# 0xPolygonZero/proof-protocol-decoder

Measured on AMD Instinct MI355X. Metric: txn-proofs/sec (whole node), 256-txn synthetic block, higher is better.
Workload: dtype u64 (Goldilocks field)

## Files before the change

include/bpg.h:

```cpp
#ifndef BPG_H
#define BPG_H
#include <stddef.h>
#include <stdint.h>

#ifdef __cplusplus
extern "C" {
#endif

typedef enum {
  BP_OK = 0,
  BP_ERR_ABORTED = -1,
  BP_ERR_INVALID_INPUT = -2,
  BP_ERR_RANGE = -3,
  BP_ERR_DEVICE = -4,
  BP_ERR_VERIFY = -5,
  BP_ERR_UNSUPPORTED = -6
} bp_status;

const char* bp_last_error(void);
const char* bp_version(void);
int bp_device_count(void);
int bp_use_blocking_sync(int device);
int bp_host_wait_mode(int device);


enum { BP_NTT_FWD_BR2NAT = 0, BP_NTT_INV_NAT2BR = 1, BP_NTT_FWD_NAT = 2, BP_NTT_INV_NAT = 3 };
int bp_ntt_batch(uint64_t* d_cols, uint32_t log_n, uint32_t n_cols, uint64_t col_stride, int dir,
                 void* stream);

int bp_intt_batch(const uint64_t* d_values, uint64_t in_stride, uint64_t* d_coeffs_out, uint64_t out_stride,
                  uint32_t log_n, uint32_t n_cols, void* stream);

int bp_lde_batch(const uint64_t* d_in, uint64_t in_stride, uint64_t* d_coeffs_out, uint64_t coeffs_stride,
                 uint64_t* d_lde_out, uint64_t lde_stride, uint32_t log_n, uint32_t rate_bits,
                 uint32_t n_cols, int from_coeffs, void* stream);

int bp_debug_copy_u64(const uint64_t* d_in, uint64_t* d_out, uint64_t n, void* stream);

int bp_debug_field_ops(const uint64_t* d_a, const uint64_t* d_b, uint64_t* d_out, uint64_t n, void* stream);

void bp_tune_quad_threshold(uint64_t n_perms);
void bp_tune_merkle_fused(int mode);
void bp_tune_merkle_wide(int log2_parents);
void bp_tune_poseidon_mx(int on);
void bp_tune_poseidon_mx_sets(int sets);
void bp_tune_poseidon_grouped(int mode);
void bp_tune_assume_loaded(int mode);
void bp_tune_rec_batch(int n);
void bp_tune_side_lanes(int n);
void bp_tune_witness_threads(int n);
void bp_tune_host_wait(int mode);
void bp_tune_host_poseidon(int mode);
int bp_debug_poseidon_host(uint64_t* states, size_t n);
void bp_tune_k5_spread(int on);
uint32_t bp_debug_poseidon_group_ops(uint32_t K);
int bp_debug_poseidon_group_tables(uint32_t K, uint32_t r0, uint8_t* out_ops, int32_t* out_cform, int32_t* out_cmain,
                                   int32_t* out_max_plane_sum);

void bp_tune_ntt_split(int mode);
void bp_tune_ntt_persist(int on, int resident_workgroups);
void bp_tune_ntt_mx(int mode);
void bp_tune_ntt_mx_wg_per_cu(int n);
int bp_debug_ntt_mx_tables(int kind, int inverse, uint8_t* out_a, int32_t* out_c, uint64_t* out_tw256,
                           uint64_t* out_tw16);
int bp_debug_poseidon_mx_cin(uint32_t* out);

int bp_poseidon_perm_batch(uint64_t* d_states, uint64_t n, void* stream);

uint64_t bp_merkle_digest_words(uint32_t log_leaves, uint32_t cap_height);
int bp_merkle_commit(const uint64_t* d_lde, uint64_t lde_stride, uint32_t n_cols, uint32_t log_n,
                     uint32_t rate_bits, uint32_t cap_height, uint64_t* d_digests, void* stream);

struct bp_stark_cfg;
typedef struct bp_air_family {
  uint32_t first_index, count;
  uint32_t kind;
  uint32_t degree;
} bp_air_family;
typedef struct bp_air_desc {
  uint32_t air_id;
  char name[24];
  uint32_t fixed_n_cols;
  uint32_t n_const_max;
  uint32_t degree;
  uint32_t n_cols, n_aux;
  uint32_t n_air_constraints, n_ctl_constraints;
  uint32_t n_units;
  uint32_t n_families;
  bp_air_family families[24];
} bp_air_desc;
uint32_t bp_air_count(void);
int bp_air_describe(uint32_t air_id, uint32_t n_cols, uint32_t n_const, uint32_t deg_pow, bp_air_desc* out);

int bp_air_register(const uint64_t* program, size_t n_words, uint32_t* air_id_out);
int bp_air_unregister(uint32_t air_id);
int bp_air_program_digest(uint32_t air_id, uint8_t out[32]);

uint64_t bp_quotient_scratch_words(uint32_t air_id, const struct bp_stark_cfg* shape);
int bp_quotient_eval(uint32_t air_id, const struct bp_stark_cfg* shape, const uint64_t* d_trace_lde,
                     const uint64_t* d_aux_lde, const uint64_t* d_const_lde, const uint64_t ctl[4],
                     const uint64_t alphas[2], uint64_t* d_scratch, uint64_t* d_qvals_out, void* stream);

typedef struct bp_air_violation {
  uint32_t row, constraint, family, kind;
  uint64_t value;
} bp_air_violation;
int bp_air_check_trace(uint32_t air_id, const struct bp_stark_cfg* shape, const uint64_t* d_trace, uint64_t stride,
                       const uint64_t* d_consts, const uint64_t pub[4], uint32_t max_rows, uint64_t* n_violated_rows,
                       uint32_t* rows_out, bp_air_violation* viol_out, uint32_t max_viol, uint32_t* n_viol, void* stream);
int bp_air_check_trace_host(uint32_t air_id, const struct bp_stark_cfg* shape, const uint64_t* trace, uint64_t stride,
                            const uint64_t* consts, const uint64_t pub[4], uint32_t max_rows, uint64_t* n_violated_rows,
                            uint32_t* rows_out, bp_air_violation* viol_out, uint32_t max_viol, uint32_t* n_viol);

int bp_keccak_trace(const uint64_t* d_inputs, uint64_t seed, uint32_t log_n, uint64_t* d_trace_out, void* stream);
int bp_logic_trace(const uint64_t* d_inputs, uint64_t seed, uint32_t log_n, uint64_t* d_trace_out, void* stream);
int bp_memory_trace(const uint64_t* d_inputs, uint64_t seed, uint32_t log_n, uint64_t* d_trace_out, void* stream);
int bp_arithmetic_trace(const uint64_t* d_inputs, uint64_t seed, uint32_t log_n, uint64_t* d_trace_out, void* stream);
int bp_byte_packing_trace(const uint64_t* d_inputs, uint64_t seed, uint32_t log_n, uint64_t* d_trace_out, void* stream);
int bp_keccak_sponge_trace(const uint64_t* d_inputs, uint64_t seed, uint32_t log_n, uint64_t* d_trace_out, void* stream);
int bp_arithmetic_mul_trace(const uint64_t* d_inputs, uint64_t seed, uint32_t log_n, uint64_t* d_trace_out, void* stream);

typedef struct bp_plonk_layout {
// ... 194 lines not shown
```

proof_protocol_decoder_amd/_lib.py:

```python
import ctypes as C
import os

_HERE = os.path.dirname(os.path.abspath(__file__))
_PATH = os.environ.get("BPG_LIBBPG") or os.path.join(_HERE, "lib", "libbpg.so")

BP_OK = 0
STATUS_NAMES = {0: "BP_OK", -1: "BP_ERR_ABORTED", -2: "BP_ERR_INVALID_INPUT", -3: "BP_ERR_RANGE",
                -4: "BP_ERR_DEVICE", -5: "BP_ERR_VERIFY", -6: "BP_ERR_UNSUPPORTED"}


class BpgError(RuntimeError):

    def __init__(self, code, message):
        super().__init__("%s: %s" % (STATUS_NAMES.get(code, str(code)), message))
        self.code = code
        self.message = message


class StarkCfg(C.Structure):
    _fields_ = [(n, C.c_uint32) for n in ("log_n", "n_cols", "n_const", "deg_pow", "rate_bits", "cap_height",
                                           "num_queries", "pow_bits", "arity_bits", "final_poly_bits")]


class AirFamily(C.Structure):
    _fields_ = [(n, C.c_uint32) for n in ("first_index", "count", "kind", "degree")]


class AirDesc(C.Structure):
    _fields_ = ([("air_id", C.c_uint32), ("name", C.c_char * 24)]
                + [(n, C.c_uint32) for n in ("fixed_n_cols", "n_const_max", "degree", "n_cols", "n_aux",
                                             "n_air_constraints", "n_ctl_constraints", "n_units", "n_families")]
                + [("families", AirFamily * 24)])


class AirViolation(C.Structure):
    _fields_ = [(n, C.c_uint32) for n in ("row", "constraint", "family", "kind")] + [("value", C.c_uint64)]


def take_buffer(ptr, length):
    try:
        return C.string_at(ptr, length.value)
    finally:
        lib().bp_free_buffer(ptr)


def lib_path():
    return _PATH


_lib = None


def lib():
    global _lib
    if _lib is not None:
        return _lib
    if not os.path.exists(_PATH):
        raise ImportError(
            "libbpg.so not built at %s -- run `python -c 'import __graft_entry__ as g; g.build()'` "
            "(hipcc --offload-arch=gfx950). There is no CPU fallback for the hot path." % _PATH)
    L = C.CDLL(_PATH)
    vp, u32, u64, i = C.c_void_p, C.c_uint32, C.c_uint64, C.c_int
    L.bp_last_error.restype = C.c_char_p
    L.bp_version.restype = C.c_char_p
    L.bp_device_count.restype = i
    L.bp_ntt_batch.argtypes = [vp, u32, u32, u64, i, vp]
    L.bp_lde_batch.argtypes = [vp, u64, vp, u64, vp, u64, u32, u32, u32, i, vp]
    L.bp_poseidon_perm_batch.argtypes = [vp, u64, vp]
    L.bp_debug_field_ops.argtypes = [vp, vp, vp, u64, vp]
    L.bp_quotient_scratch_words.argtypes = [u32, C.POINTER(StarkCfg)]
    L.bp_quotient_scratch_words.restype = u64
    L.bp_quotient_eval.argtypes = [u32, C.POINTER(StarkCfg), vp, vp, vp, C.POINTER(u64), C.POINTER(u64), vp, vp, vp]
    L.bp_air_count.restype = u32
    L.bp_air_describe.argtypes = [u32, u32, u32, u32, C.POINTER(AirDesc)]
    check_args = [u32, C.POINTER(StarkCfg), vp, u64, vp, C.POINTER(u64), u32, C.POINTER(u64), C.POINTER(u32),
                  C.POINTER(AirViolation), u32, C.POINTER(u32)]
    L.bp_air_check_trace.argtypes = check_args + [vp]
    L.bp_air_check_trace_host.argtypes = check_args
    L.bp_keccak_trace.argtypes = [vp, u64, u32, vp, vp]
    L.bp_logic_trace.argtypes = [vp, u64, u32, vp, vp]
    L.bp_memory_trace.argtypes = [vp, u64, u32, vp, vp]
    L.bp_arithmetic_trace.argtypes = [vp, u64, u32, vp, vp]
    L.bp_byte_packing_trace.argtypes = [vp, u64, u32, vp, vp]
    L.bp_keccak_sponge_trace.argtypes = [vp, u64, u32, vp, vp]
    L.bp_arithmetic_mul_trace.argtypes = [vp, u64, u32, vp, vp]
    L.bp_stark_verify_air.argtypes = [u32, C.POINTER(StarkCfg), C.POINTER(u64), C.c_char_p, C.c_size_t]
    L.bp_stark_prove_air.argtypes = [u32, C.POINTER(StarkCfg), u64, u64, i, C.POINTER(C.POINTER(C.c_uint8)),
                                     C.POINTER(C.c_size_t)]
    L.bp_stark_verify_air_pub.argtypes = [u32, C.POINTER(StarkCfg), C.POINTER(u64), C.POINTER(u64), C.c_char_p, C.c_size_t]
    L.bp_stark_prove_trace.argtypes = [u32, C.POINTER(StarkCfg), vp, u64, vp, C.POINTER(u64), i, C.POINTER(C.POINTER(C.c_uint8)),
                                       C.POINTER(C.c_size_t)]
    L.bp_air_register.argtypes = [vp, C.c_size_t, C.POINTER(u32)]
    L.bp_air_unregister.argtypes = [u32]
    L.bp_air_program_digest.argtypes = [u32, C.c_char_p]
    L.bp_fri_fold.argtypes = [vp, u32, u32, u32, u64, C.POINTER(u64), vp, vp]
    L.bp_openings.argtypes = [vp, u64, u32, u32, C.POINTER(u64), C.POINTER(u64), vp, vp, vp]
    L.bp_pow_grind.argtypes = [C.POINTER(u64), u32, u32, C.POINTER(u64), vp]
    L.bp_merkle_digest_words.argtypes = [u32, u32]
    L.bp_merkle_digest_words.restype = u64
    L.bp_merkle_commit.argtypes = [vp, u64, u32, u32, u32, u32, vp, vp]
    L.bp_stark_prove_synthetic.argtypes = [C.POINTER(StarkCfg), u64, u64, i, C.POINTER(C.POINTER(C.c_uint8)),
                                           C.POINTER(C.c_size_t)]
    L.bp_free_buffer.argtypes = [C.POINTER(C.c_uint8)]
    L.bp_free_buffer.restype = None
    L.bp_tune_quad_threshold.argtypes = [u64]
    L.bp_tune_quad_threshold.restype = None
    L.bp_tune_ntt_mx.argtypes = [i]
    L.bp_tune_ntt_mx.restype = None
    L.bp_tune_ntt_mx_wg_per_cu.argtypes = [i]
    L.bp_tune_ntt_mx_wg_per_cu.restype = None
    L.bp_tune_poseidon_mx.argtypes = [i]
    L.bp_tune_poseidon_mx.restype = None
    L.bp_tune_poseidon_mx_sets.argtypes = [i]
    L.bp_tune_poseidon_mx_sets.restype = None
    _lib = L
    return L


def check(rc):
    if rc != BP_OK:
        raise BpgError(rc, lib().bp_last_error().decode("utf-8", "replace"))
```

proof_protocol_decoder_amd/csrc/gl.hpp:

```cpp
#pragma once
#include <cstdint>
#include <hip/hip_runtime.h>

#define GL_HD __host__ __device__ __forceinline__

namespace gl {

constexpr uint64_t P = 0xFFFFFFFF00000001ULL;
constexpr uint64_t EPS = 0xFFFFFFFFULL;
constexpr uint64_t GENERATOR = 7;
constexpr uint64_t TWO_ADIC_ROOT = 1753635133440165772ULL;
constexpr uint64_t W = 7;

#if defined(__HIP__)
namespace cc {
typedef uint64_t mask;
__device__ __forceinline__ uint64_t mad_co(uint32_t a, uint32_t b, uint64_t c, mask& co) {
  uint64_t d;
  asm("v_mad_u64_u32 %0, %1, %2, %3, %4" : "=v"(d), "=s"(co) : "v"(a), "v"(b), "v"(c));
  return d;
}
__device__ __forceinline__ uint64_t mad_eps_co(uint32_t a, uint64_t c, mask& co) {
  uint64_t d;
  asm("v_mad_u64_u32 %0, %1, %2, -1, %3" : "=v"(d), "=s"(co) : "v"(a), "v"(c));
  return d;
}
__device__ __forceinline__ uint32_t add_co(uint32_t a, uint32_t b, mask& co) {
  uint32_t d;
  asm("v_add_co_u32_e64 %0, %1, %2, %3" : "=v"(d), "=s"(co) : "v"(a), "v"(b));
  return d;
}
__device__ __forceinline__ uint32_t addc_co(uint32_t a, uint32_t b, mask ci, mask& co) {
  uint32_t d;
  asm("s_nop 1\n\tv_addc_co_u32_e64 %0, %1, %2, %3, %4" : "=v"(d), "=s"(co) : "v"(a), "v"(b), "s"(ci));
  return d;
}
__device__ __forceinline__ uint32_t addc0_co(uint32_t a, mask ci, mask& co) {
  uint32_t d;
  asm("s_nop 1\n\tv_addc_co_u32_e64 %0, %1, %2, 0, %3" : "=v"(d), "=s"(co) : "v"(a), "s"(ci));
  return d;
}
__device__ __forceinline__ uint32_t sub_co(uint32_t a, uint32_t b, mask& co) {
  uint32_t d;
  asm("v_sub_co_u32_e64 %0, %1, %2, %3" : "=v"(d), "=s"(co) : "v"(a), "v"(b));
  return d;
}
__device__ __forceinline__ uint32_t subb_co(uint32_t a, uint32_t b, mask ci, mask& co) {
  uint32_t d;
  asm("s_nop 1\n\tv_subb_co_u32_e64 %0, %1, %2, %3, %4" : "=v"(d), "=s"(co) : "v"(a), "v"(b), "s"(ci));
  return d;
}
__device__ __forceinline__ uint32_t subb0_co(uint32_t a, mask ci, mask& co) {
  uint32_t d;
  asm("s_nop 1\n\tv_subbrev_co_u32_e64 %0, %1, 0, %2, %3" : "=v"(d), "=s"(co) : "v"(a), "s"(ci));
  return d;
}
__device__ __forceinline__ uint32_t sel_eps(mask m) {
  uint32_t d;
  asm("s_nop 1\n\tv_cndmask_b32_e64 %0, 0, -1, %1" : "=v"(d) : "s"(m));
  return d;
}
__device__ __forceinline__ uint64_t mk64(uint32_t lo, uint32_t hi) { return ((uint64_t)hi << 32) | lo; }
#include "gl_cc.inc"
}
#endif
GL_HD uint64_t canon(uint64_t a) {
  return a >= P ? a - P : a;
}

GL_HD uint64_t add(uint64_t a, uint64_t b) {
  uint64_t s = a + b;
  return s < b ? s + EPS : s;
}
GL_HD uint64_t sub(uint64_t a, uint64_t b) {
  uint64_t d = a - b;
  return a < b ? d - EPS : d;
}
GL_HD uint64_t addc(uint64_t a, uint64_t b) {
  uint64_t s = a + b;
  return (s < a || s >= P) ? s - P : s;
}
GL_HD uint64_t subc(uint64_t a, uint64_t b) {
  return a >= b ? a - b : a + (P - b);
}
GL_HD uint64_t negc(uint64_t a) {
  return a ? P - a : 0;
}

GL_HD uint64_t reduce128(uint64_t lo, uint64_t hi) {
  uint64_t hh = hi >> 32, hl = hi & EPS;
  uint64_t t0 = lo - hh;
  if (lo < hh) t0 -= EPS;
  uint64_t t1 = (hl << 32) - hl;
  uint64_t r = t0 + t1;
  return r < t1 ? r + EPS : r;
}

GL_HD void mul_wide(uint64_t a, uint64_t b, uint64_t& lo, uint64_t& hi) {
#if defined(__HIP_DEVICE_COMPILE__)
  uint32_t a0 = (uint32_t)a, a1 = (uint32_t)(a >> 32), b0 = (uint32_t)b, b1 = (uint32_t)(b >> 32);
  uint64_t p00 = (uint64_t)a0 * b0;
  uint64_t mid = (uint64_t)a0 * b1 + (p00 >> 32);
  uint64_t mid2 = (uint64_t)a1 * b0 + (uint32_t)mid;
  hi = (uint64_t)a1 * b1 + (mid >> 32) + (mid2 >> 32);
  lo = (mid2 << 32) | (uint32_t)p00;
#else
  unsigned __int128 x = (unsigned __int128)a * b;
// ... 41 lines not shown
    P[i] = (uint64_t)a0 * b0[i];
    M[i] = (uint64_t)a0 * b1;
    Q[i] = (uint64_t)a1[i] * b1;
  }
  cc::mad_co(M, C, a1, b0);
#pragma unroll
  for (int i = 0; i < N; i++) {
    t0[i] = (uint32_t)P[i]; t1[i] = (uint32_t)(P[i] >> 32); m0[i] = (uint32_t)M[i]; m1[i] = (uint32_t)(M[i] >> 32);
    q0[i] = (uint32_t)Q[i]; q1[i] = (uint32_t)(Q[i] >> 32);
  }
  cc::add_co(t1, c1, m0);
  cc::addc_co(m1, c2, q0, c1);
  cc::addc0_cv(q1, C);
#pragma unroll
  for (int i = 0; i < N; i++) P[i] = cc::mk64(t0[i], t1[i]);
  cc::mad_eps_co(P, c3, m1);
#pragma unroll
  for (int i = 0; i < N; i++) { t0[i] = (uint32_t)P[i]; t1[i] = (uint32_t)(P[i] >> 32); }
  cc::subb0_co(t0, b3, c3);
#pragma unroll
  for (int i = 0; i < N; i++) c3[i] &= ~b3[i];
  cc::addc0_cv(t1, c3);
  cc::subb_co(t0, bw, q1, c2);
  cc::subb0_co(t1, bw2, bw);
  cc::addc0_co(t0, b3, bw2);
#pragma unroll
  for (int i = 0; i < N; i++) bw2[i] &= ~b3[i];
  cc::subb0_cv(t1, bw2);
#pragma unroll
  for (int i = 0; i < N; i++) r[i] = cc::mk64(t0[i], t1[i]);
}
#endif
#if defined(__HIP__)
template <int N>
__device__ __forceinline__ void add_n(const uint64_t (&a)[N], const uint64_t (&b)[N], uint64_t (&r)[N]) {
  uint32_t al[N], ah[N], bl[N], bh[N], lo[N], hi[N];
  cc::mask c1[N], c2[N], c3[N];
#pragma unroll
  for (int i = 0; i < N; i++) {
    al[i] = (uint32_t)a[i]; ah[i] = (uint32_t)(a[i] >> 32); bl[i] = (uint32_t)b[i]; bh[i] = (uint32_t)(b[i] >> 32);
  }
  cc::add_co_o(lo, c1, al, bl);
  cc::addc_co_o(hi, c2, ah, bh, c1);
  cc::subb0_co(lo, c3, c2);
#pragma unroll
  for (int i = 0; i < N; i++) c2[i] &= ~c3[i];
  cc::addc0_cv(hi, c2);
#pragma unroll
  for (int i = 0; i < N; i++) r[i] = cc::mk64(lo[i], hi[i]);
}
template <int N>
__device__ __forceinline__ void sub_n(const uint64_t (&a)[N], const uint64_t (&b)[N], uint64_t (&r)[N]) {
  uint32_t al[N], ah[N], bl[N], bh[N], lo[N], hi[N];
  cc::mask b1[N], b2[N], b3[N];
#pragma unroll
  for (int i = 0; i < N; i++) {
    al[i] = (uint32_t)a[i]; ah[i] = (uint32_t)(a[i] >> 32); bl[i] = (uint32_t)b[i]; bh[i] = (uint32_t)(b[i] >> 32);
  }
  cc::sub_co_o(lo, b1, al, bl);
  cc::subb_co_o(hi, b2, ah, bh, b1);
  cc::addc0_co(lo, b3, b2);
#pragma unroll
  for (int i = 0; i < N; i++) b2[i] &= ~b3[i];
  cc::subb0_cv(hi, b2);
#pragma unroll
  for (int i = 0; i < N; i++) r[i] = cc::mk64(lo[i], hi[i]);
}
template <int N>
__device__ __forceinline__ void canon_n(uint64_t (&a)[N]) {
  uint32_t lo[N], hi[N], tl[N], th[N];
  cc::mask k[N], c[N];
#pragma unroll
  for (int i = 0; i < N; i++) {
    lo[i] = (uint32_t)a[i]; hi[i] = (uint32_t)(a[i] >> 32);
  }
  cc::add_m1_co_o(tl, k, lo);
  cc::addc0_co_o(th, c, hi, k);
  cc::sel(lo, tl, c);
  cc::sel(hi, th, c);
#pragma unroll
  for (int i = 0; i < N; i++) a[i] = cc::mk64(lo[i], hi[i]);
}
#endif
#if defined(__HIP__)
struct DotAcc {
  uint64_t p, m, q;
  uint32_t cp, cm, cq;
};
__device__ __forceinline__ DotAcc dot_zero() { return DotAcc{0, 0, 0, 0, 0, 0}; }
__device__ __forceinline__ void dot_mad4(DotAcc (&acc)[4], const uint64_t (&a)[4], const uint64_t (&b)[4]) {
  uint32_t a0[4], a1[4], b0[4], b1[4], cnt[4];
  uint64_t col[4];
  cc::mask c[4], cx[4];
#pragma unroll
  for (int i = 0; i < 4; i++) {
    a0[i] = (uint32_t)a[i]; a1[i] = (uint32_t)(a[i] >> 32); b0[i] = (uint32_t)b[i]; b1[i] = (uint32_t)(b[i] >> 32);
  }
#define BPG_DOT_COL(COL, CNT, X, Y)                                  \
  _Pragma("unroll") for (int i = 0; i < 4; i++) { col[i] = acc[i].COL; cnt[i] = acc[i].CNT; } \
  cc::mad_co(col, c, X, Y);                                           \
  cc::addc0_co(cnt, cx, c);                                           \
  _Pragma("unroll") for (int i = 0; i < 4; i++) { acc[i].COL = col[i]; acc[i].CNT = cnt[i]; }
  BPG_DOT_COL(p, cp, a0, b0)
  BPG_DOT_COL(m, cm, a0, b1)
  BPG_DOT_COL(m, cm, a1, b0)
  BPG_DOT_COL(q, cq, a1, b1)
#undef BPG_DOT_COL
}
GL_HD uint64_t mulc(uint64_t a, uint64_t b);
GL_HD uint64_t addc(uint64_t a, uint64_t b);
__device__ __forceinline__ uint64_t dot_reduce(const DotAcc& d) {
  uint64_t r = canon(d.p);
  r = addc(r, mulc(d.m, (uint64_t)1 << 32));
  r = addc(r, mulc(d.q, EPS));
  r = addc(r, mulc(d.cp, EPS));
  r = subc(r, canon((uint64_t)d.cm));
  r = subc(r, mulc(d.cq, (uint64_t)1 << 32));
  return r;
}
#endif
GL_HD uint64_t sqr(uint64_t a) { return mul(a, a); }
GL_HD uint64_t mulc(uint64_t a, uint64_t b) { return canon(mul(a, b)); }

GL_HD uint64_t pow(uint64_t a, uint64_t e) {
  uint64_t r = 1;
  while (e) {
    if (e & 1) r = mulc(r, a);
    a = mulc(a, a);
    e >>= 1;
  }
  return r;
}
GL_HD uint64_t inv(uint64_t a) {
  auto sq_n = [](uint64_t x, int n) {
    for (int i = 0; i < n; i++) x = mul(x, x);
    return x;
  };
  const uint64_t e1 = a;
  const uint64_t e2 = mul(sq_n(e1, 1), e1);
  const uint64_t e3 = mul(sq_n(e2, 1), e1);
  const uint64_t e6 = mul(sq_n(e3, 3), e3);
  const uint64_t e12 = mul(sq_n(e6, 6), e6);
  const uint64_t e24 = mul(sq_n(e12, 12), e12);
  const uint64_t e30 = mul(sq_n(e24, 6), e6);
  const uint64_t e31 = mul(sq_n(e30, 1), e1);
  const uint64_t hi = sq_n(e31, 1);
  const uint64_t lo = mul(hi, a);
  return mulc(sq_n(hi, 32), lo);
}
GL_HD uint64_t root(unsigned k) {
  uint64_t r = TWO_ADIC_ROOT;
  for (unsigned i = k; i < 32; i++) r = mulc(r, r);
  return r;
}

struct Ext {
  uint64_t c0, c1;
};
GL_HD Ext ext(uint64_t a, uint64_t b = 0) { return Ext{a, b}; }
GL_HD bool eq(Ext a, Ext b) { return a.c0 == b.c0 && a.c1 == b.c1; }
GL_HD Ext add(Ext a, Ext b) { return Ext{addc(a.c0, b.c0), addc(a.c1, b.c1)}; }
GL_HD Ext sub(Ext a, Ext b) { return Ext{subc(a.c0, b.c0), subc(a.c1, b.c1)}; }
GL_HD uint64_t mul7(uint64_t x) {
  const uint64_t p = (uint64_t)(uint32_t)x * 7u;
  const uint64_t m = (x >> 32) * 7u + (p >> 32);
  const uint64_t u = (m << 32) | (uint32_t)p;
// ... 43 lines not shown
```

proof_protocol_decoder_amd/csrc/gl_cc.inc:

```
__device__ __forceinline__ void mad_co(uint64_t (&x)[3], mask (&co)[3], const uint32_t (&a)[3], const uint32_t (&b)[3]) {
  asm("v_mad_u64_u32 %0, %3, %6, %9, %0\n\tv_mad_u64_u32 %1, %4, %7, %10, %1\n\tv_mad_u64_u32 %2, %5, %8, %11, %2"
      : "+v"(x[0]), "+v"(x[1]), "+v"(x[2]), "=&s"(co[0]), "=&s"(co[1]), "=&s"(co[2])
      : "v"(a[0]), "v"(a[1]), "v"(a[2]), "v"(b[0]), "v"(b[1]), "v"(b[2]));
}
__device__ __forceinline__ void mad_eps_co(uint64_t (&x)[3], mask (&co)[3], const uint32_t (&a)[3]) {
  asm("v_mad_u64_u32 %0, %3, %6, -1, %0\n\tv_mad_u64_u32 %1, %4, %7, -1, %1\n\tv_mad_u64_u32 %2, %5, %8, -1, %2"
      : "+v"(x[0]), "+v"(x[1]), "+v"(x[2]), "=&s"(co[0]), "=&s"(co[1]), "=&s"(co[2])
      : "v"(a[0]), "v"(a[1]), "v"(a[2]));
}
__device__ __forceinline__ void add_co(uint32_t (&x)[3], mask (&co)[3], const uint32_t (&b)[3]) {
  asm("v_add_co_u32_e64 %0, %3, %0, %6\n\tv_add_co_u32_e64 %1, %4, %1, %7\n\tv_add_co_u32_e64 %2, %5, %2, %8"
      : "+v"(x[0]), "+v"(x[1]), "+v"(x[2]), "=&s"(co[0]), "=&s"(co[1]), "=&s"(co[2])
      : "v"(b[0]), "v"(b[1]), "v"(b[2]));
}
__device__ __forceinline__ void addc_co(uint32_t (&x)[3], mask (&co)[3], const uint32_t (&b)[3], const mask (&ci)[3]) {
  asm("v_addc_co_u32_e64 %0, %3, %0, %6, %9\n\tv_addc_co_u32_e64 %1, %4, %1, %7, %10\n\tv_addc_co_u32_e64 %2, %5, %2, %8, %11"
      : "+v"(x[0]), "+v"(x[1]), "+v"(x[2]), "=&s"(co[0]), "=&s"(co[1]), "=&s"(co[2])
      : "v"(b[0]), "v"(b[1]), "v"(b[2]), "s"(ci[0]), "s"(ci[1]), "s"(ci[2]));
}
__device__ __forceinline__ void addc0_co(uint32_t (&x)[3], mask (&co)[3], const mask (&ci)[3]) {
  asm("v_addc_co_u32_e64 %0, %3, %0, 0, %6\n\tv_addc_co_u32_e64 %1, %4, %1, 0, %7\n\tv_addc_co_u32_e64 %2, %5, %2, 0, %8"
      : "+v"(x[0]), "+v"(x[1]), "+v"(x[2]), "=&s"(co[0]), "=&s"(co[1]), "=&s"(co[2])
      : "s"(ci[0]), "s"(ci[1]), "s"(ci[2]));
}
// ... 2 lines not shown
      : "+v"(x[0]), "+v"(x[1]), "+v"(x[2]), "=&s"(co[0]), "=&s"(co[1]), "=&s"(co[2])
      : "v"(b[0]), "v"(b[1]), "v"(b[2]));
}
__device__ __forceinline__ void subb_co(uint32_t (&x)[3], mask (&co)[3], const uint32_t (&b)[3], const mask (&ci)[3]) {
  asm("v_subb_co_u32_e64 %0, %3, %0, %6, %9\n\tv_subb_co_u32_e64 %1, %4, %1, %7, %10\n\tv_subb_co_u32_e64 %2, %5, %2, %8, %11"
      : "+v"(x[0]), "+v"(x[1]), "+v"(x[2]), "=&s"(co[0]), "=&s"(co[1]), "=&s"(co[2])
      : "v"(b[0]), "v"(b[1]), "v"(b[2]), "s"(ci[0]), "s"(ci[1]), "s"(ci[2]));
}
__device__ __forceinline__ void subb0_co(uint32_t (&x)[3], mask (&co)[3], const mask (&ci)[3]) {
  asm("v_subbrev_co_u32_e64 %0, %3, 0, %0, %6\n\tv_subbrev_co_u32_e64 %1, %4, 0, %1, %7\n\tv_subbrev_co_u32_e64 %2, %5, 0, %2, %8"
      : "+v"(x[0]), "+v"(x[1]), "+v"(x[2]), "=&s"(co[0]), "=&s"(co[1]), "=&s"(co[2])
      : "s"(ci[0]), "s"(ci[1]), "s"(ci[2]));
}
__device__ __forceinline__ void add_m1_co(uint32_t (&x)[3], mask (&co)[3]) {
  asm("v_add_co_u32_e64 %0, %3, %0, -1\n\tv_add_co_u32_e64 %1, %4, %1, -1\n\tv_add_co_u32_e64 %2, %5, %2, -1"
      : "+v"(x[0]), "+v"(x[1]), "+v"(x[2]), "=&s"(co[0]), "=&s"(co[1]), "=&s"(co[2])
      : );
}
__device__ __forceinline__ void sel(uint32_t (&x)[3], const uint32_t (&b)[3], const mask (&ci)[3]) {
  asm("v_cndmask_b32_e64 %0, %0, %3, %6\n\tv_cndmask_b32_e64 %1, %1, %4, %7\n\tv_cndmask_b32_e64 %2, %2, %5, %8"
      : "+v"(x[0]), "+v"(x[1]), "+v"(x[2])
      : "v"(b[0]), "v"(b[1]), "v"(b[2]), "s"(ci[0]), "s"(ci[1]), "s"(ci[2]));
}
__device__ __forceinline__ void sel_eps(uint32_t (&x)[3], const mask (&ci)[3]) {
  asm("v_cndmask_b32_e64 %0, 0, -1, %3\n\tv_cndmask_b32_e64 %1, 0, -1, %4\n\tv_cndmask_b32_e64 %2, 0, -1, %5"
      : "=&v"(x[0]), "=&v"(x[1]), "=&v"(x[2])
      : "s"(ci[0]), "s"(ci[1]), "s"(ci[2]));
}
__device__ __forceinline__ void addc0_cv(uint32_t (&x)[3], const mask (&ci)[3]) {
  asm("v_addc_co_u32_e64 %0, vcc, %0, 0, %3\n\tv_addc_co_u32_e64 %1, vcc, %1, 0, %4\n\tv_addc_co_u32_e64 %2, vcc, %2, 0, %5"
      : "+v"(x[0]), "+v"(x[1]), "+v"(x[2])
      : "s"(ci[0]), "s"(ci[1]), "s"(ci[2]) : "vcc");
}
__device__ __forceinline__ void addc_cv(uint32_t (&x)[3], const uint32_t (&b)[3], const mask (&ci)[3]) {
  asm("v_addc_co_u32_e64 %0, vcc, %0, %3, %6\n\tv_addc_co_u32_e64 %1, vcc, %1, %4, %7\n\tv_addc_co_u32_e64 %2, vcc, %2, %5, %8"
      : "+v"(x[0]), "+v"(x[1]), "+v"(x[2])
      : "v"(b[0]), "v"(b[1]), "v"(b[2]), "s"(ci[0]), "s"(ci[1]), "s"(ci[2]) : "vcc");
}
__device__ __forceinline__ void subb0_cv(uint32_t (&x)[3], const mask (&ci)[3]) {
  asm("v_subbrev_co_u32_e64 %0, vcc, 0, %0, %3\n\tv_subbrev_co_u32_e64 %1, vcc, 0, %1, %4\n\tv_subbrev_co_u32_e64 %2, vcc, 0, %2, %5"
      : "+v"(x[0]), "+v"(x[1]), "+v"(x[2])
      : "s"(ci[0]), "s"(ci[1]), "s"(ci[2]) : "vcc");
}
__device__ __forceinline__ void mad_eps_cv(uint64_t (&x)[3], const uint32_t (&a)[3]) {
  asm("v_mad_u64_u32 %0, vcc, %3, -1, %0\n\tv_mad_u64_u32 %1, vcc, %4, -1, %1\n\tv_mad_u64_u32 %2, vcc, %5, -1, %2"
      : "+v"(x[0]), "+v"(x[1]), "+v"(x[2])
      : "v"(a[0]), "v"(a[1]), "v"(a[2]) : "vcc");
}
__device__ __forceinline__ void sel_one(uint32_t (&x)[3], const mask (&ci)[3]) {
  asm("v_cndmask_b32_e64 %0, %0, 1, %3\n\tv_cndmask_b32_e64 %1, %1, 1, %4\n\tv_cndmask_b32_e64 %2, %2, 1, %5"
      : "+v"(x[0]), "+v"(x[1]), "+v"(x[2])
      : "s"(ci[0]), "s"(ci[1]), "s"(ci[2]));
}
__device__ __forceinline__ void add_co_o(uint32_t (&x)[3], mask (&co)[3], const uint32_t (&a)[3], const uint32_t (&b)[3]) {
  asm("v_add_co_u32_e64 %0, %3, %6, %9\n\tv_add_co_u32_e64 %1, %4, %7, %10\n\tv_add_co_u32_e64 %2, %5, %8, %11"
      : "=&v"(x[0]), "=&v"(x[1]), "=&v"(x[2]), "=&s"(co[0]), "=&s"(co[1]), "=&s"(co[2])
      : "v"(a[0]), "v"(a[1]), "v"(a[2]), "v"(b[0]), "v"(b[1]), "v"(b[2]));
}
__device__ __forceinline__ void addc_co_o(uint32_t (&x)[3], mask (&co)[3], const uint32_t (&a)[3], const uint32_t (&b)[3], const mask (&ci)[3]) {
  asm("v_addc_co_u32_e64 %0, %3, %6, %9, %12\n\tv_addc_co_u32_e64 %1, %4, %7, %10, %13\n\tv_addc_co_u32_e64 %2, %5, %8, %11, %14"
      : "=&v"(x[0]), "=&v"(x[1]), "=&v"(x[2]), "=&s"(co[0]), "=&s"(co[1]), "=&s"(co[2])
      : "v"(a[0]), "v"(a[1]), "v"(a[2]), "v"(b[0]), "v"(b[1]), "v"(b[2]), "s"(ci[0]), "s"(ci[1]), "s"(ci[2]));
}
__device__ __forceinline__ void sub_co_o(uint32_t (&x)[3], mask (&co)[3], const uint32_t (&a)[3], const uint32_t (&b)[3]) {
  asm("v_sub_co_u32_e64 %0, %3, %6, %9\n\tv_sub_co_u32_e64 %1, %4, %7, %10\n\tv_sub_co_u32_e64 %2, %5, %8, %11"
      : "=&v"(x[0]), "=&v"(x[1]), "=&v"(x[2]), "=&s"(co[0]), "=&s"(co[1]), "=&s"(co[2])
      : "v"(a[0]), "v"(a[1]), "v"(a[2]), "v"(b[0]), "v"(b[1]), "v"(b[2]));
}
__device__ __forceinline__ void subb_co_o(uint32_t (&x)[3], mask (&co)[3], const uint32_t (&a)[3], const uint32_t (&b)[3], const mask (&ci)[3]) {
  asm("v_subb_co_u32_e64 %0, %3, %6, %9, %12\n\tv_subb_co_u32_e64 %1, %4, %7, %10, %13\n\tv_subb_co_u32_e64 %2, %5, %8, %11, %14"
      : "=&v"(x[0]), "=&v"(x[1]), "=&v"(x[2]), "=&s"(co[0]), "=&s"(co[1]), "=&s"(co[2])
      : "v"(a[0]), "v"(a[1]), "v"(a[2]), "v"(b[0]), "v"(b[1]), "v"(b[2]), "s"(ci[0]), "s"(ci[1]), "s"(ci[2]));
}
__device__ __forceinline__ void add_m1_co_o(uint32_t (&x)[3], mask (&co)[3], const uint32_t (&a)[3]) {
  asm("v_add_co_u32_e64 %0, %3, %6, -1\n\tv_add_co_u32_e64 %1, %4, %7, -1\n\tv_add_co_u32_e64 %2, %5, %8, -1"
      : "=&v"(x[0]), "=&v"(x[1]), "=&v"(x[2]), "=&s"(co[0]), "=&s"(co[1]), "=&s"(co[2])
      : "v"(a[0]), "v"(a[1]), "v"(a[2]));
}
__device__ __forceinline__ void addc0_co_o(uint32_t (&x)[3], mask (&co)[3], const uint32_t (&a)[3], const mask (&ci)[3]) {
  asm("v_addc_co_u32_e64 %0, %3, %6, 0, %9\n\tv_addc_co_u32_e64 %1, %4, %7, 0, %10\n\tv_addc_co_u32_e64 %2, %5, %8, 0, %11"
      : "=&v"(x[0]), "=&v"(x[1]), "=&v"(x[2]), "=&s"(co[0]), "=&s"(co[1]), "=&s"(co[2])
      : "v"(a[0]), "v"(a[1]), "v"(a[2]), "s"(ci[0]), "s"(ci[1]), "s"(ci[2]));
}
__device__ __forceinline__ void mad_co(uint64_t (&x)[4], mask (&co)[4], const uint32_t (&a)[4], const uint32_t (&b)[4]) {
  asm("v_mad_u64_u32 %0, %4, %8, %12, %0\n\tv_mad_u64_u32 %1, %5, %9, %13, %1\n\tv_mad_u64_u32 %2, %6, %10, %14, %2\n\tv_mad_u64_u32 %3, %7, %11, %15, %3"
      : "+v"(x[0]), "+v"(x[1]), "+v"(x[2]), "+v"(x[3]), "=&s"(co[0]), "=&s"(co[1]), "=&s"(co[2]), "=&s"(co[3])
      : "v"(a[0]), "v"(a[1]), "v"(a[2]), "v"(a[3]), "v"(b[0]), "v"(b[1]), "v"(b[2]), "v"(b[3]));
}
__device__ __forceinline__ void mad_eps_co(uint64_t (&x)[4], mask (&co)[4], const uint32_t (&a)[4]) {
  asm("v_mad_u64_u32 %0, %4, %8, -1, %0\n\tv_mad_u64_u32 %1, %5, %9, -1, %1\n\tv_mad_u64_u32 %2, %6, %10, -1, %2\n\tv_mad_u64_u32 %3, %7, %11, -1, %3"
      : "+v"(x[0]), "+v"(x[1]), "+v"(x[2]), "+v"(x[3]), "=&s"(co[0]), "=&s"(co[1]), "=&s"(co[2]), "=&s"(co[3])
      : "v"(a[0]), "v"(a[1]), "v"(a[2]), "v"(a[3]));
}
__device__ __forceinline__ void add_co(uint32_t (&x)[4], mask (&co)[4], const uint32_t (&b)[4]) {
  asm("v_add_co_u32_e64 %0, %4, %0, %8\n\tv_add_co_u32_e64 %1, %5, %1, %9\n\tv_add_co_u32_e64 %2, %6, %2, %10\n\tv_add_co_u32_e64 %3, %7, %3, %11"
      : "+v"(x[0]), "+v"(x[1]), "+v"(x[2]), "+v"(x[3]), "=&s"(co[0]), "=&s"(co[1]), "=&s"(co[2]), "=&s"(co[3])
      : "v"(b[0]), "v"(b[1]), "v"(b[2]), "v"(b[3]));
}
__device__ __forceinline__ void addc_co(uint32_t (&x)[4], mask (&co)[4], const uint32_t (&b)[4], const mask (&ci)[4]) {
  asm("v_addc_co_u32_e64 %0, %4, %0, %8, %12\n\tv_addc_co_u32_e64 %1, %5, %1, %9, %13\n\tv_addc_co_u32_e64 %2, %6, %2, %10, %14\n\tv_addc_co_u32_e64 %3, %7, %3, %11, %15"
      : "+v"(x[0]), "+v"(x[1]), "+v"(x[2]), "+v"(x[3]), "=&s"(co[0]), "=&s"(co[1]), "=&s"(co[2]), "=&s"(co[3])
      : "v"(b[0]), "v"(b[1]), "v"(b[2]), "v"(b[3]), "s"(ci[0]), "s"(ci[1]), "s"(ci[2]), "s"(ci[3]));
}
__device__ __forceinline__ void addc0_co(uint32_t (&x)[4], mask (&co)[4], const mask (&ci)[4]) {
  asm("v_addc_co_u32_e64 %0, %4, %0, 0, %8\n\tv_addc_co_u32_e64 %1, %5, %1, 0, %9\n\tv_addc_co_u32_e64 %2, %6, %2, 0, %10\n\tv_addc_co_u32_e64 %3, %7, %3, 0, %11"
      : "+v"(x[0]), "+v"(x[1]), "+v"(x[2]), "+v"(x[3]), "=&s"(co[0]), "=&s"(co[1]), "=&s"(co[2]), "=&s"(co[3])
      : "s"(ci[0]), "s"(ci[1]), "s"(ci[2]), "s"(ci[3]));
}
__device__ __forceinline__ void sub_co(uint32_t (&x)[4], mask (&co)[4], const uint32_t (&b)[4]) {
  asm("v_sub_co_u32_e64 %0, %4, %0, %8\n\tv_sub_co_u32_e64 %1, %5, %1, %9\n\tv_sub_co_u32_e64 %2, %6, %2, %10\n\tv_sub_co_u32_e64 %3, %7, %3, %11"
      : "+v"(x[0]), "+v"(x[1]), "+v"(x[2]), "+v"(x[3]), "=&s"(co[0]), "=&s"(co[1]), "=&s"(co[2]), "=&s"(co[3])
      : "v"(b[0]), "v"(b[1]), "v"(b[2]), "v"(b[3]));
}
__device__ __forceinline__ void subb_co(uint32_t (&x)[4], mask (&co)[4], const uint32_t (&b)[4], const mask (&ci)[4]) {
  asm("v_subb_co_u32_e64 %0, %4, %0, %8, %12\n\tv_subb_co_u32_e64 %1, %5, %1, %9, %13\n\tv_subb_co_u32_e64 %2, %6, %2, %10, %14\n\tv_subb_co_u32_e64 %3, %7, %3, %11, %15"
      : "+v"(x[0]), "+v"(x[1]), "+v"(x[2]), "+v"(x[3]), "=&s"(co[0]), "=&s"(co[1]), "=&s"(co[2]), "=&s"(co[3])
      : "v"(b[0]), "v"(b[1]), "v"(b[2]), "v"(b[3]), "s"(ci[0]), "s"(ci[1]), "s"(ci[2]), "s"(ci[3]));
}
__device__ __forceinline__ void subb0_co(uint32_t (&x)[4], mask (&co)[4], const mask (&ci)[4]) {
  asm("v_subbrev_co_u32_e64 %0, %4, 0, %0, %8\n\tv_subbrev_co_u32_e64 %1, %5, 0, %1, %9\n\tv_subbrev_co_u32_e64 %2, %6, 0, %2, %10\n\tv_subbrev_co_u32_e64 %3, %7, 0, %3, %11"
      : "+v"(x[0]), "+v"(x[1]), "+v"(x[2]), "+v"(x[3]), "=&s"(co[0]), "=&s"(co[1]), "=&s"(co[2]), "=&s"(co[3])
      : "s"(ci[0]), "s"(ci[1]), "s"(ci[2]), "s"(ci[3]));
}
__device__ __forceinline__ void add_m1_co(uint32_t (&x)[4], mask (&co)[4]) {
  asm("v_add_co_u32_e64 %0, %4, %0, -1\n\tv_add_co_u32_e64 %1, %5, %1, -1\n\tv_add_co_u32_e64 %2, %6, %2, -1\n\tv_add_co_u32_e64 %3, %7, %3, -1"
      : "+v"(x[0]), "+v"(x[1]), "+v"(x[2]), "+v"(x[3]), "=&s"(co[0]), "=&s"(co[1]), "=&s"(co[2]), "=&s"(co[3])
      : );
}
__device__ __forceinline__ void sel(uint32_t (&x)[4], const uint32_t (&b)[4], const mask (&ci)[4]) {
  asm("v_cndmask_b32_e64 %0, %0, %4, %8\n\tv_cndmask_b32_e64 %1, %1, %5, %9\n\tv_cndmask_b32_e64 %2, %2, %6, %10\n\tv_cndmask_b32_e64 %3, %3, %7, %11"
      : "+v"(x[0]), "+v"(x[1]), "+v"(x[2]), "+v"(x[3])
      : "v"(b[0]), "v"(b[1]), "v"(b[2]), "v"(b[3]), "s"(ci[0]), "s"(ci[1]), "s"(ci[2]), "s"(ci[3]));
}
__device__ __forceinline__ void sel_eps(uint32_t (&x)[4], const mask (&ci)[4]) {
  asm("v_cndmask_b32_e64 %0, 0, -1, %4\n\tv_cndmask_b32_e64 %1, 0, -1, %5\n\tv_cndmask_b32_e64 %2, 0, -1, %6\n\tv_cndmask_b32_e64 %3, 0, -1, %7"
      : "=&v"(x[0]), "=&v"(x[1]), "=&v"(x[2]), "=&v"(x[3])
      : "s"(ci[0]), "s"(ci[1]), "s"(ci[2]), "s"(ci[3]));
}
__device__ __forceinline__ void addc0_cv(uint32_t (&x)[4], const mask (&ci)[4]) {
  asm("v_addc_co_u32_e64 %0, vcc, %0, 0, %4\n\tv_addc_co_u32_e64 %1, vcc, %1, 0, %5\n\tv_addc_co_u32_e64 %2, vcc, %2, 0, %6\n\tv_addc_co_u32_e64 %3, vcc, %3, 0, %7"
      : "+v"(x[0]), "+v"(x[1]), "+v"(x[2]), "+v"(x[3])
      : "s"(ci[0]), "s"(ci[1]), "s"(ci[2]), "s"(ci[3]) : "vcc");
}
__device__ __forceinline__ void addc_cv(uint32_t (&x)[4], const uint32_t (&b)[4], const mask (&ci)[4]) {
  asm("v_addc_co_u32_e64 %0, vcc, %0, %4, %8\n\tv_addc_co_u32_e64 %1, vcc, %1, %5, %9\n\tv_addc_co_u32_e64 %2, vcc, %2, %6, %10\n\tv_addc_co_u32_e64 %3, vcc, %3, %7, %11"
      : "+v"(x[0]), "+v"(x[1]), "+v"(x[2]), "+v"(x[3])
      : "v"(b[0]), "v"(b[1]), "v"(b[2]), "v"(b[3]), "s"(ci[0]), "s"(ci[1]), "s"(ci[2]), "s"(ci[3]) : "vcc");
}
__device__ __forceinline__ void subb0_cv(uint32_t (&x)[4], const mask (&ci)[4]) {
  asm("v_subbrev_co_u32_e64 %0, vcc, 0, %0, %4\n\tv_subbrev_co_u32_e64 %1, vcc, 0, %1, %5\n\tv_subbrev_co_u32_e64 %2, vcc, 0, %2, %6\n\tv_subbrev_co_u32_e64 %3, vcc, 0, %3, %7"
      : "+v"(x[0]), "+v"(x[1]), "+v"(x[2]), "+v"(x[3])
      : "s"(ci[0]), "s"(ci[1]), "s"(ci[2]), "s"(ci[3]) : "vcc");
}
__device__ __forceinline__ void mad_eps_cv(uint64_t (&x)[4], const uint32_t (&a)[4]) {
  asm("v_mad_u64_u32 %0, vcc, %4, -1, %0\n\tv_mad_u64_u32 %1, vcc, %5, -1, %1\n\tv_mad_u64_u32 %2, vcc, %6, -1, %2\n\tv_mad_u64_u32 %3, vcc, %7, -1, %3"
      : "+v"(x[0]), "+v"(x[1]), "+v"(x[2]), "+v"(x[3])
      : "v"(a[0]), "v"(a[1]), "v"(a[2]), "v"(a[3]) : "vcc");
}
__device__ __forceinline__ void sel_one(uint32_t (&x)[4], const mask (&ci)[4]) {
  asm("v_cndmask_b32_e64 %0, %0, 1, %4\n\tv_cndmask_b32_e64 %1, %1, 1, %5\n\tv_cndmask_b32_e64 %2, %2, 1, %6\n\tv_cndmask_b32_e64 %3, %3, 1, %7"
      : "+v"(x[0]), "+v"(x[1]), "+v"(x[2]), "+v"(x[3])
      : "s"(ci[0]), "s"(ci[1]), "s"(ci[2]), "s"(ci[3]));
}
__device__ __forceinline__ void add_co_o(uint32_t (&x)[4], mask (&co)[4], const uint32_t (&a)[4], const uint32_t (&b)[4]) {
  asm("v_add_co_u32_e64 %0, %4, %8, %12\n\tv_add_co_u32_e64 %1, %5, %9, %13\n\tv_add_co_u32_e64 %2, %6, %10, %14\n\tv_add_co_u32_e64 %3, %7, %11, %15"
      : "=&v"(x[0]), "=&v"(x[1]), "=&v"(x[2]), "=&v"(x[3]), "=&s"(co[0]), "=&s"(co[1]), "=&s"(co[2]), "=&s"(co[3])
      : "v"(a[0]), "v"(a[1]), "v"(a[2]), "v"(a[3]), "v"(b[0]), "v"(b[1]), "v"(b[2]), "v"(b[3]));
}
__device__ __forceinline__ void addc_co_o(uint32_t (&x)[4], mask (&co)[4], const uint32_t (&a)[4], const uint32_t (&b)[4], const mask (&ci)[4]) {
  asm("v_addc_co_u32_e64 %0, %4, %8, %12, %16\n\tv_addc_co_u32_e64 %1, %5, %9, %13, %17\n\tv_addc_co_u32_e64 %2, %6, %10, %14, %18\n\tv_addc_co_u32_e64 %3, %7, %11, %15, %19"
      : "=&v"(x[0]), "=&v"(x[1]), "=&v"(x[2]), "=&v"(x[3]), "=&s"(co[0]), "=&s"(co[1]), "=&s"(co[2]), "=&s"(co[3])
      : "v"(a[0]), "v"(a[1]), "v"(a[2]), "v"(a[3]), "v"(b[0]), "v"(b[1]), "v"(b[2]), "v"(b[3]), "s"(ci[0]), "s"(ci[1]), "s"(ci[2]), "s"(ci[3]));
}
__device__ __forceinline__ void sub_co_o(uint32_t (&x)[4], mask (&co)[4], const uint32_t (&a)[4], const uint32_t (&b)[4]) {
  asm("v_sub_co_u32_e64 %0, %4, %8, %12\n\tv_sub_co_u32_e64 %1, %5, %9, %13\n\tv_sub_co_u32_e64 %2, %6, %10, %14\n\tv_sub_co_u32_e64 %3, %7, %11, %15"
      : "=&v"(x[0]), "=&v"(x[1]), "=&v"(x[2]), "=&v"(x[3]), "=&s"(co[0]), "=&s"(co[1]), "=&s"(co[2]), "=&s"(co[3])
      : "v"(a[0]), "v"(a[1]), "v"(a[2]), "v"(a[3]), "v"(b[0]), "v"(b[1]), "v"(b[2]), "v"(b[3]));
}
__device__ __forceinline__ void subb_co_o(uint32_t (&x)[4], mask (&co)[4], const uint32_t (&a)[4], const uint32_t (&b)[4], const mask (&ci)[4]) {
  asm("v_subb_co_u32_e64 %0, %4, %8, %12, %16\n\tv_subb_co_u32_e64 %1, %5, %9, %13, %17\n\tv_subb_co_u32_e64 %2, %6, %10, %14, %18\n\tv_subb_co_u32_e64 %3, %7, %11, %15, %19"
      : "=&v"(x[0]), "=&v"(x[1]), "=&v"(x[2]), "=&v"(x[3]), "=&s"(co[0]), "=&s"(co[1]), "=&s"(co[2]), "=&s"(co[3])
      : "v"(a[0]), "v"(a[1]), "v"(a[2]), "v"(a[3]), "v"(b[0]), "v"(b[1]), "v"(b[2]), "v"(b[3]), "s"(ci[0]), "s"(ci[1]), "s"(ci[2]), "s"(ci[3]));
}
__device__ __forceinline__ void add_m1_co_o(uint32_t (&x)[4], mask (&co)[4], const uint32_t (&a)[4]) {
  asm("v_add_co_u32_e64 %0, %4, %8, -1\n\tv_add_co_u32_e64 %1, %5, %9, -1\n\tv_add_co_u32_e64 %2, %6, %10, -1\n\tv_add_co_u32_e64 %3, %7, %11, -1"
      : "=&v"(x[0]), "=&v"(x[1]), "=&v"(x[2]), "=&v"(x[3]), "=&s"(co[0]), "=&s"(co[1]), "=&s"(co[2]), "=&s"(co[3])
      : "v"(a[0]), "v"(a[1]), "v"(a[2]), "v"(a[3]));
}
__device__ __forceinline__ void addc0_co_o(uint32_t (&x)[4], mask (&co)[4], const uint32_t (&a)[4], const mask (&ci)[4]) {
  asm("v_addc_co_u32_e64 %0, %4, %8, 0, %12\n\tv_addc_co_u32_e64 %1, %5, %9, 0, %13\n\tv_addc_co_u32_e64 %2, %6, %10, 0, %14\n\tv_addc_co_u32_e64 %3, %7, %11, 0, %15"
      : "=&v"(x[0]), "=&v"(x[1]), "=&v"(x[2]), "=&v"(x[3]), "=&s"(co[0]), "=&s"(co[1]), "=&s"(co[2]), "=&s"(co[3])
      : "v"(a[0]), "v"(a[1]), "v"(a[2]), "v"(a[3]), "s"(ci[0]), "s"(ci[1]), "s"(ci[2]), "s"(ci[3]));
}
```

proof_protocol_decoder_amd/csrc/hash_kernels.hip:

```cpp
#include <atomic>
#include <cstring>
#include <memory>
#include <mutex>
#include <vector>
#include "common.hpp"
#include "poseidon.cuh"
#include "poseidon_mx.cuh"
#include "stark_kernels.hpp"

namespace {

__global__ void __launch_bounds__(256) perm_batch_kernel(uint64_t* __restrict__ states, uint64_t n) {
  uint64_t i = blockIdx.x * (uint64_t)blockDim.x + threadIdx.x;
  if (i >= n) return;
  uint64_t s[12];
#pragma unroll
  for (int k = 0; k < 12; k++) s[k] = states[i * 12 + k];
  poseidon::permute(s);
#pragma unroll
  for (int k = 0; k < 12; k++) states[i * 12 + k] = gl::canon(s[k]);
}

__global__ void __launch_bounds__(256) __attribute__((amdgpu_waves_per_eu(4, 8)))
leaf_hash_kernel(const uint64_t* __restrict__ lde, uint64_t stride, uint32_t n_cols, uint32_t log_n,
// ... 327 lines not shown
        if (mirror && l + 1 == levels) mirror[(wg_first + q) * 4 + c.kb] = d;
        sm[l & 1][q * 4 + c.kb] = d;
      }
    }
    __syncthreads();
    dst += level_parents * 4;
    level_parents >>= 1;
    wg_parents >>= 1;
    wg_first >>= 1;
  }
}

__global__ void __launch_bounds__(256)
merkle_subtree_wide_kernel(const uint64_t* __restrict__ child, uint64_t* __restrict__ out, uint64_t n_parents,
                           uint32_t levels, uint64_t* __restrict__ mirror, uint64_t dig_bstride) {
  if (gridDim.x * gridDim.z <= 64) __builtin_amdgcn_s_setprio(3);
  child += blockIdx.z * dig_bstride;
  out += blockIdx.z * dig_bstride;
  if (mirror) mirror += blockIdx.z * ((n_parents >> (levels - 1)) * 4);
  __shared__ __attribute__((aligned(16))) uint32_t cin[poseidon::mx::CIN_WORDS];
  __shared__ uint64_t sm[2][256 * 4];
  poseidon::mx::build_cin(cin);
  __syncthreads();
  const poseidon::mx::Ctx c = poseidon::mx::make_ctx(cin);
  const uint32_t wave = threadIdx.x >> 6, n = threadIdx.x & 15;
  uint64_t level_parents = n_parents;
  uint32_t wg_parents = n_parents < 256 ? (uint32_t)n_parents : 256u;
  uint64_t wg_first = (uint64_t)blockIdx.x * 256;
  uint64_t* dst = out;
  for (uint32_t l = 0; l < levels; l++) {
    const uint64_t* prev = sm[(l - 1) & 1];
    if (wg_parents >= 64) {
      if (wave * 64 < wg_parents) {
        uint64_t e[4][3];
#pragma unroll
        for (int m = 0; m < 4; m++) {
          const uint32_t q = wave * 64 + 16 * m + n;
          if (l == 0) {
            e[m][0] = child[(wg_first + q) * 8 + c.kb];
            e[m][1] = child[(wg_first + q) * 8 + 4 + c.kb];
          } else {
            e[m][0] = prev[(2 * q) * 4 + c.kb];
            e[m][1] = prev[(2 * q + 1) * 4 + c.kb];
          }
          e[m][2] = 0;
        }
        poseidon::mx::permute<4>(e, c);
#pragma unroll
        for (int m = 0; m < 4; m++) {
          const uint32_t q = wave * 64 + 16 * m + n;
          const uint64_t d = gl::canon(e[m][0]);
          dst[(wg_first + q) * 4 + c.kb] = d;
          if (mirror && l + 1 == levels) mirror[(wg_first + q) * 4 + c.kb] = d;
          sm[l & 1][q * 4 + c.kb] = d;
        }
      }
    } else if (wave * 16 < wg_parents) {
      const uint32_t q = wave * 16 + n, qc = q < wg_parents ? q : wg_parents - 1;
      uint64_t e[1][3];
      if (l == 0) {
        e[0][0] = child[(wg_first + qc) * 8 + c.kb];
        e[0][1] = child[(wg_first + qc) * 8 + 4 + c.kb];
      } else {
        e[0][0] = prev[(2 * qc) * 4 + c.kb];
        e[0][1] = prev[(2 * qc + 1) * 4 + c.kb];
      }
      e[0][2] = 0;
      poseidon::mx::permute<1>(e, c);
      if (q < wg_parents) {
        const uint64_t d = gl::canon(e[0][0]);
        dst[(wg_first + q) * 4 + c.kb] = d;
        if (mirror && l + 1 == levels) mirror[(wg_first + q) * 4 + c.kb] = d;
        sm[l & 1][q * 4 + c.kb] = d;
      }
    }
    __syncthreads();
    dst += level_parents * 4;
    level_parents >>= 1;
    wg_parents >>= 1;
    wg_first >>= 1;
  }
}

__global__ void __launch_bounds__(256)
calib_copy_u64_kernel(const uint64_t* __restrict__ in, uint64_t* __restrict__ out, uint64_t n) {
  uint64_t i = blockIdx.x * (uint64_t)blockDim.x + threadIdx.x;
  const uint64_t stride = (uint64_t)gridDim.x * blockDim.x;
  for (; i < n; i += stride) out[i] = in[i];
}

__global__ void __launch_bounds__(256) field_ops_kernel(const uint64_t* __restrict__ a, const uint64_t* __restrict__ b,
                                                        uint64_t* __restrict__ out, uint64_t n) {
  const uint64_t i0 = (blockIdx.x * (uint64_t)blockDim.x + threadIdx.x) * 4;
  if (i0 >= n) return;
  uint64_t x[4], y[4];
#pragma unroll
  for (int k = 0; k < 4; k++) {
    const uint64_t i = i0 + k < n ? i0 + k : n - 1;
    x[k] = a[i];
    y[k] = b[i];
  }
  uint64_t r4[4], r3[3];
  gl::mul_n<4>(x, y, r4);
  __builtin_amdgcn_sched_barrier(0);
  const uint64_t x3[3] = {x[1], x[2], x[3]}, y3[3] = {y[1], y[2], y[3]};
  gl::mul_n<3>(x3, y3, r3);
  __builtin_amdgcn_sched_barrier(0);
  gl::DotAcc d[4] = {gl::dot_zero(), gl::dot_zero(), gl::dot_zero(), gl::dot_zero()};
  gl::dot_mad4(d, x, y);
  __builtin_amdgcn_sched_barrier(0);
  gl::dot_mad4(d, y, x);
  __builtin_amdgcn_sched_barrier(0);
  const uint64_t yy[4] = {y[0], y[0], y[0], y[0]};
  gl::dot_mad4(d, x, yy);
  __builtin_amdgcn_sched_barrier(0);
  uint64_t cy[4] = {y[0], y[1], y[2], y[3]}, sum4[4], dif4[4], cx4[4] = {x[0], x[1], x[2], x[3]};
  gl::canon_n<4>(cy);
  __builtin_amdgcn_sched_barrier(0);
  gl::add_n<4>(x, cy, sum4);
  __builtin_amdgcn_sched_barrier(0);
  gl::sub_n<4>(x, cy, dif4);
  __builtin_amdgcn_sched_barrier(0);
  gl::canon_n<4>(cx4);
  __builtin_amdgcn_sched_barrier(0);
#pragma unroll
  for (int k = 0; k < 4; k++) {
    const uint64_t i = i0 + k;
    if (i >= n) break;
    const uint64_t cb = gl::canon(y[k]);
    out[0 * n + i] = gl::canon(gl::mul(x[k], y[k]));
    out[1 * n + i] = gl::canon(r4[k]);
    out[2 * n + i] = k ? gl::canon(r3[k - 1]) : gl::canon(r4[0]);
    uint64_t lo, hi;
    gl::mul_wide(x[k], y[k], lo, hi);
    out[3 * n + i] = gl::canon(gl::reduce128(lo, hi));
    out[4 * n + i] = gl::canon(gl::add(x[k], cb));
    out[5 * n + i] = gl::canon(gl::sub(x[k], cb));
    out[6 * n + i] = gl::dot_reduce(d[k]);
    out[7 * n + i] = gl::canon(gl::mul7(x[k]));
    out[8 * n + i] = gl::inv(gl::canon(x[k]));
    const gl::Ext e = gl::mul(gl::Ext{gl::canon(x[k]), cb}, gl::Ext{cb, gl::canon(x[k] ^ y[k])});
    out[9 * n + i] = e.c0;
    out[10 * n + i] = e.c1;
    out[11 * n + i] = gl::canon(sum4[k]);
    out[12 * n + i] = gl::canon(dif4[k]);
    out[13 * n + i] = cx4[k];
    out[14 * n + i] = cy[k];
  }
}

}

namespace bpg {


static std::atomic<uint64_t> g_quad_threshold{0};
static bool g_poseidon_mx_on();
static std::atomic<int> g_active_provers{0};
void prover_active(int delta) { g_active_provers.fetch_add(delta, std::memory_order_relaxed); }
int provers_active() { return g_active_provers.load(std::memory_order_relaxed); }
static std::atomic<int> g_assume_loaded{-1};
bool device_loaded() {
  const int a = g_assume_loaded.load(std::memory_order_relaxed);
  return a < 0 ? g_active_provers.load(std::memory_order_relaxed) >= 6 : a != 0;
}
uint64_t quad_threshold() {
// ... 110 lines not shown
  uint64_t* lvl = d_digests;
  uint32_t l = log_leaves;
  if (mirrored) *mirrored = false;
  if (batch == 0 || batch > MAX_BATCH) return fail(BP_ERR_INVALID_INPUT, "merkle: batch of %u trees", batch);
  while (l > cap_height) {
    const uint64_t cnt = (uint64_t)1 << l, parents = cnt / 2;
    uint64_t* nxt = lvl + cnt * 4;
    const int fmode = g_merkle_fused.load(std::memory_order_relaxed);
    const uint64_t flimit = fmode >= 8 ? (uint64_t)1 << fmode : 2048;
    const bool fused = parents <= flimit && (parents < quad_threshold() || fmode >= 8) && (fmode > 0 || (fmode < 0 && !device_loaded()));
    const uint64_t wlimit = (uint64_t)1 << g_merkle_wide_log2.load(std::memory_order_relaxed);
    if (!fused && fmode > 0 && poseidon_mx() && parents >= 256 && parents <= wlimit && parents % 256 == 0) {
      uint32_t levels = l - cap_height;
      if (levels > 9) levels = 9;
      uint64_t* mir = (l - levels == cap_height) ? mirror : nullptr;
      merkle_subtree_wide_kernel<<<dim3((uint32_t)(parents / 256), 1, batch), 256, 0, st>>>(lvl, nxt, parents, levels, mir, dig_bstride);
      BPG_LAUNCH_CHECK();
      if (mir && mirrored) *mirrored = true;
      for (uint32_t k = 0; k < levels; k++) {
        lvl += ((uint64_t)1 << l) * 4;
        l--;
      }
      continue;
    }
    if (!fused) {
      uint64_t* mir = (l - 1 == cap_height) ? mirror : nullptr;
      if (const int ns = mx_sets(parents * batch)) {
        BPG_MX_DISPATCH(ns, merkle_level_mx_kernel, parents, batch, lvl, nxt, parents, mir, dig_bstride)
      } else if (parents * batch >= quad_threshold())
        merkle_level_kernel<<<dim3(ceil_div(parents, 256), 1, batch), 256, 0, st>>>(lvl, nxt, parents, mir, dig_bstride);
      else
        merkle_level_quad_kernel<<<dim3(ceil_div(cnt * 2, 256), 1, batch), 256, 0, st>>>(lvl, nxt, parents, mir, dig_bstride);
      BPG_LAUNCH_CHECK();
      if (mir && mirrored) *mirrored = true;
      lvl = nxt;
      l--;
      continue;
    }
    uint32_t levels = l - cap_height;
    const uint32_t wgs = parents >= 64 ? (uint32_t)(parents / 64) : 1;
    uint32_t max_levels = 1;
    for (uint64_t p = parents >= 64 ? 64 : parents; p > 1; p >>= 1) max_levels++;
    if (levels > max_levels) levels = max_levels;
    uint64_t* mir = (l - levels == cap_height) ? mirror : nullptr;
    if (poseidon_mx()) merkle_subtree_mx_kernel<<<dim3(wgs, 1, batch), 256, 0, st>>>(lvl, nxt, parents, levels, mir, dig_bstride);
    else merkle_subtree_quad_kernel<<<dim3(wgs, 1, batch), 256, 0, st>>>(lvl, nxt, parents, levels, mir, dig_bstride);
    BPG_LAUNCH_CHECK();
    if (mir && mirrored) *mirrored = true;
    for (uint32_t k = 0; k < levels; k++) {
      lvl += ((uint64_t)1 << l) * 4;
      l--;
    }
  }
  return BP_OK;
}

int merkle_commit_rows(const uint64_t* d_leaves, uint32_t leaf_len, uint32_t log_leaves, uint32_t cap_height,
                       uint64_t* d_digests, hipStream_t st) {
  uint64_t n = (uint64_t)1 << log_leaves;
  leaf_hash_rows_kernel<<<ceil_div(n, 256), 256, 0, st>>>(d_leaves, leaf_len, n, d_digests);
  BPG_LAUNCH_CHECK();
  return merkle_upper_levels(d_digests, log_leaves, cap_height, st, nullptr, nullptr);
}

}

extern "C" {

int bp_debug_copy_u64(const uint64_t* d_in, uint64_t* d_out, uint64_t n, void* stream) {
  if (!d_in || !d_out) return bpg::fail(BP_ERR_INVALID_INPUT, "bp_debug_copy_u64: null buffer");
  calib_copy_u64_kernel<<<4096, 256, 0, bpg::as_stream(stream)>>>(d_in, d_out, n);
  BPG_LAUNCH_CHECK();
  return BP_OK;
}

int bp_debug_field_ops(const uint64_t* d_a, const uint64_t* d_b, uint64_t* d_out, uint64_t n, void* stream) {
  if (!n) return BP_OK;
  if (!d_a || !d_b || !d_out) return bpg::fail(BP_ERR_INVALID_INPUT, "bp_debug_field_ops: null buffer");
  field_ops_kernel<<<bpg::ceil_div(bpg::ceil_div(n, 4), 256), 256, 0, bpg::as_stream(stream)>>>(d_a, d_b, d_out, n);
  BPG_LAUNCH_CHECK();
  return BP_OK;
}

void bp_tune_merkle_fused(int mode) { bpg::g_merkle_fused.store(mode < 0 ? -1 : (mode >= 8 && mode <= 20 ? mode : (mode != 0))); }
void bp_tune_quad_threshold(uint64_t n_perms) { bpg::g_quad_threshold.store(n_perms); }
void bp_tune_poseidon_mx(int on) { bpg::g_poseidon_mx.store(on != 0); }
int bp_debug_poseidon_mx_cin(uint32_t* out) {
  if (!out) return bpg::fail(BP_ERR_INVALID_INPUT, "bp_debug_poseidon_mx_cin: null buffer");
  static const poseidon::mx::CinTable t = poseidon::mx::make_cin_table();
  for (int i = 0; i < poseidon::mx::CIN_WORDS; i++) out[i] = t.v[i];
  return BP_OK;
}
void bp_tune_merkle_wide(int log2_parents) { bpg::g_merkle_wide_log2.store(log2_parents < 8 || log2_parents > 24 ? 0 : log2_parents); }
void bp_tune_assume_loaded(int mode) { bpg::g_assume_loaded.store(mode < 0 ? -1 : (mode != 0)); }
void bp_tune_poseidon_grouped(int mode) { bpg::g_poseidon_grouped.store(mode == 0 ? 0 : (mode == 2 ? 2 : 3)); }

uint32_t bp_debug_poseidon_group_ops(uint32_t K) { return K >= 2 && K <= 8 ? (uint32_t)poseidon::group::layout((int)K).n_ops : 0; }
int bp_debug_poseidon_group_tables(uint32_t K, uint32_t r0, uint8_t* out_ops, int32_t* out_cform, int32_t* out_cmain,
                                   int32_t* out_max_plane_sum) try {
  if (!out_ops || !out_cform || !out_cmain) return bpg::fail(BP_ERR_INVALID_INPUT, "bp_debug_poseidon_group_tables: null output");
  poseidon::group::Tables t;
  if (!poseidon::group::build((int)K, (int)r0, &t))
    return bpg::fail(BP_ERR_INVALID_INPUT, "bp_debug_poseidon_group_tables: no such group (K=%u r0=%u)", K, r0);
  std::memcpy(out_ops, t.ops.data(), t.ops.size());
  std::memcpy(out_cform, t.cform.data(), t.cform.size() * 4);
  std::memcpy(out_cmain, t.cmain.data(), t.cmain.size() * 4);
  if (out_max_plane_sum) *out_max_plane_sum = t.max_plane_sum;
  return BP_OK;
}
BPG_ABI_CATCH("bp_debug_poseidon_group_tables")

void bp_tune_poseidon_mx_sets(int sets) { bpg::g_mx_sets.store(sets == 1 || sets == 2 || sets == 4 ? sets : 0); }

uint64_t bp_merkle_digest_words(uint32_t log_leaves, uint32_t cap_height) {
  return (((uint64_t)2 << log_leaves) - ((uint64_t)1 << cap_height)) * 4;
}

int bp_poseidon_perm_batch(uint64_t* d_states, uint64_t n, void* stream) try {
  if (!n) return BP_OK;
  if (!d_states) return bpg::fail(BP_ERR_INVALID_INPUT, "bp_poseidon_perm_batch: null buffer");
  hipStream_t st = bpg::as_stream(stream);
  using bpg::ceil_div;
  if (const int ns = bpg::mx_sets(n)) {
    BPG_MX_DISPATCH(ns, perm_batch_mx_kernel, n, 1, d_states, n)
  } else
    perm_batch_kernel<<<bpg::ceil_div(n, 256), 256, 0, st>>>(d_states, n);
  BPG_LAUNCH_CHECK();
  return BP_OK;
}
BPG_ABI_CATCH("bp_poseidon_perm_batch")

int bp_merkle_commit(const uint64_t* d_lde, uint64_t lde_stride, uint32_t n_cols, uint32_t log_n,
                     uint32_t rate_bits, uint32_t cap_height, uint64_t* d_digests, void* stream) try {
  return bpg::merkle_commit_cols(d_lde, lde_stride, n_cols, log_n, rate_bits, cap_height, d_digests,
                                 bpg::as_stream(stream), nullptr, nullptr, 1, 0, 0);
}
BPG_ABI_CATCH("bp_merkle_commit")

}

namespace bpg {

int merkle_commit_cols(const uint64_t* d_lde, uint64_t lde_stride, uint32_t n_cols, uint32_t log_n, uint32_t rate_bits,
                       uint32_t cap_height, uint64_t* d_digests, hipStream_t st, uint64_t* mirror, bool* mirrored,
                       uint32_t batch, uint64_t lde_bstride, uint64_t dig_bstride) {
  const uint32_t log_leaves = log_n + rate_bits;
  if (!d_lde || !d_digests) return fail(BP_ERR_INVALID_INPUT, "bp_merkle_commit: null buffer");
  if (log_leaves > 30 || cap_height > log_leaves || n_cols == 0 || lde_stride < ((uint64_t)1 << log_leaves))
    return fail(BP_ERR_INVALID_INPUT,
                "bp_merkle_commit: bad shape (log_n=%u rate_bits=%u cap_height=%u n_cols=%u stride=%llu)", log_n,
                rate_bits, cap_height, n_cols, (unsigned long long)lde_stride);
  if (batch == 0 || batch > MAX_BATCH) return fail(BP_ERR_INVALID_INPUT, "merkle: batch of %u trees", batch);
  uint64_t rows = (uint64_t)1 << log_leaves;
  {
    KernelTimer kt(PROF_LEAF_HASH, st, n_cols > 4 ? (double)batch * (double)rows * (double)((n_cols + 7) / 8) : 0.0);
    int ns = mx_sets(rows * batch);
    while (ns > 1 && (uint64_t)16 * ns > rows) ns >>= 1;
    if (ns && rows >= 16) {
      BPG_MX_DISPATCH(ns, leaf_hash_mx_kernel, rows, batch, d_lde, lde_stride, n_cols, log_n, rate_bits, d_digests, lde_bstride, dig_bstride)
    } else if (rows * batch < quad_threshold())
      leaf_hash_quad_kernel<<<dim3(ceil_div(rows * 4, 256), 1, batch), 256, 0, st>>>(d_lde, lde_stride, n_cols, log_n, rate_bits,
                                                                               d_digests, lde_bstride, dig_bstride);
    else
      leaf_hash_kernel<<<dim3(ceil_div(rows, 256), 1, batch), 256, 0, st>>>(d_lde, lde_stride, n_cols, log_n, rate_bits, d_digests,
                                                                      lde_bstride, dig_bstride);
  }
// ... 6 lines not shown
```

proof_protocol_decoder_amd/csrc/ntt.hip:

```cpp
#include <atomic>
#include <map>
#include <mutex>
#include <tuple>
#include <cstring>
#include <memory>
#include "common.hpp"
#include "gl.hpp"
#include "mx_arith.cuh"

namespace {

constexpr uint32_t LOG_BLK_MAX = 14;

template <int N>
__device__ __forceinline__ void mul_group(uint64_t (&x)[16], const int (&idx)[4], const uint64_t (&d)[4], const uint64_t (&w)[4]) {
  if constexpr (N == 4) {
    uint64_t r[4];
    gl::mul_n<4>(d, w, r);
#pragma unroll
    for (int i = 0; i < 4; i++) x[idx[i]] = r[i];
  } else if constexpr (N == 3) {
    const uint64_t d3[3] = {d[0], d[1], d[2]}, w3[3] = {w[0], w[1], w[2]};
    uint64_t r[3];
    gl::mul_n<3>(d3, w3, r);
#pragma unroll
    for (int i = 0; i < 3; i++) x[idx[i]] = r[i];
  } else {
#pragma unroll
    for (int i = 0; i < N; i++) x[idx[i]] = gl::mul(d[i], w[i]);
  }
}

template <int LOGR, bool J0 = false>
__device__ __forceinline__ void dif_butterflies(uint64_t (&x)[1 << LOGR], const uint64_t* __restrict__ tw,
                                                uint32_t j, uint32_t log_sub, uint32_t tw_shift) {
  constexpr int R = 1 << LOGR, NB = R / 2;
#pragma unroll
  for (int s = 0; s < LOGR; s++) {
    const int half = R >> (s + 1);
    if constexpr (NB % 4 == 0 && J0 && LOGR == 4) {
      uint64_t dd[NB];
#pragma unroll
      for (int k0 = 0; k0 < NB; k0 += 4) {
        uint64_t a[4], b[4], d[4], r[4];
#pragma unroll
        for (int i = 0; i < 4; i++) {
          const int k = k0 + i, m = (k / half) * 2 * half + (k % half);
          a[i] = x[m];
          b[i] = x[m + half];
        }
        gl::canon_n<4>(b);
        gl::add_n<4>(a, b, r);
        gl::sub_n<4>(a, b, d);
#pragma unroll
        for (int i = 0; i < 4; i++) {
          const int k = k0 + i, m = (k / half) * 2 * half + (k % half);
          x[m] = r[i];
          dd[k] = d[i];
        }
      }
      int cnt = 0;
      int idx[4] = {0, 0, 0, 0};
      uint64_t dv[4] = {0, 0, 0, 0}, wv[4] = {0, 0, 0, 0};
      uint64_t xx[16];
#pragma unroll
      for (int i = 0; i < 16; i++) xx[i] = x[i];
#pragma unroll
      for (int k = 0; k < NB; k++) {
        const int m = (k / half) * 2 * half + (k % half), e = m & (half - 1);
        if (e == 0) {
          xx[m + half] = dd[k];
        } else {
          idx[cnt] = m + half;
          dv[cnt] = dd[k];
          wv[cnt] = tw[(uint32_t)e << (tw_shift + s)];
          cnt++;
          if (cnt == 4) {
            mul_group<4>(xx, idx, dv, wv);
            cnt = 0;
          }
        }
      }
      if (cnt == 3) mul_group<3>(xx, idx, dv, wv);
      else if (cnt == 2) mul_group<2>(xx, idx, dv, wv);
      else if (cnt == 1) mul_group<1>(xx, idx, dv, wv);
#pragma unroll
      for (int i = 0; i < 16; i++) x[i] = xx[i];
    } else if constexpr (NB % 4 == 0) {
#pragma unroll
      for (int k0 = 0; k0 < NB; k0 += 4) {
        uint64_t a[4], b[4], d[4], w[4], r[4];
#pragma unroll
        for (int i = 0; i < 4; i++) {
          const int k = k0 + i, m = (k / half) * 2 * half + (k % half);
          const uint32_t p = j + ((uint32_t)(m & (half - 1)) << log_sub);
          w[i] = tw[p << (tw_shift + s)];
          a[i] = x[m];
          b[i] = x[m + half];
        }
        gl::canon_n<4>(b);
        gl::add_n<4>(a, b, r);
        gl::sub_n<4>(a, b, d);
#pragma unroll
        for (int i = 0; i < 4; i++) {
          const int k = k0 + i, m = (k / half) * 2 * half + (k % half);
          x[m] = r[i];
        }
        gl::mul_n<4>(d, w, r);
#pragma unroll
        for (int i = 0; i < 4; i++) {
          const int k = k0 + i, m = (k / half) * 2 * half + (k % half);
          x[m + half] = r[i];
        }
        if constexpr (LOGR >= 4) __builtin_amdgcn_sched_barrier(0);
      }
    } else {
#pragma unroll
      for (int m = 0; m < R; m++) {
        if (m & half) continue;
        const uint64_t a = x[m], b = gl::canon(x[m + half]);
        x[m] = gl::add(a, b);
        if (J0 && (m & (half - 1)) == 0) {
          x[m + half] = gl::sub(a, b);
        } else {
          const uint32_t p = j + ((uint32_t)(m & (half - 1)) << log_sub);
          x[m + half] = gl::mul(gl::sub(a, b), tw[p << (tw_shift + s)]);
        }
      }
    }
  }
}
template <int LOGR, bool J0 = false>
__device__ __forceinline__ void dit_butterflies(uint64_t (&x)[1 << LOGR], const uint64_t* __restrict__ tw,
                                                uint32_t j, uint32_t log_sub, uint32_t tw_shift) {
  constexpr int R = 1 << LOGR, NB = R / 2;
#pragma unroll
  for (int s = 0; s < LOGR; s++) {
    const int step = 1 << s;
    if constexpr (NB % 4 == 0 && J0 && LOGR == 4) {
      uint64_t xx[16];
#pragma unroll
      for (int i = 0; i < 16; i++) xx[i] = x[i];
      int cnt = 0;
      int idx[4] = {0, 0, 0, 0};
      uint64_t dv[4] = {0, 0, 0, 0}, wv[4] = {0, 0, 0, 0};
#pragma unroll
      for (int k = 0; k < NB; k++) {
        const int m = (k / step) * 2 * step + (k % step), e = m & (step - 1);
        if (e != 0) {
          idx[cnt] = m + step;
          dv[cnt] = x[m + step];
          wv[cnt] = tw[(uint32_t)e << (tw_shift + (LOGR - 1 - s))];
          cnt++;
          if (cnt == 4) {
            mul_group<4>(xx, idx, dv, wv);
            cnt = 0;
          }
        }
      }
      if (cnt == 3) mul_group<3>(xx, idx, dv, wv);
      else if (cnt == 2) mul_group<2>(xx, idx, dv, wv);
      else if (cnt == 1) mul_group<1>(xx, idx, dv, wv);
#pragma unroll
      for (int k0 = 0; k0 < NB; k0 += 4) {
        uint64_t a[4], r[4], hi[4], lo[4];
#pragma unroll
        for (int i = 0; i < 4; i++) {
          const int k = k0 + i, m = (k / step) * 2 * step + (k % step);
          a[i] = xx[m];
          r[i] = xx[m + step];
        }
        gl::canon_n<4>(r);
        gl::add_n<4>(a, r, hi);
        gl::sub_n<4>(a, r, lo);
#pragma unroll
        for (int i = 0; i < 4; i++) {
          const int k = k0 + i, m = (k / step) * 2 * step + (k % step);
          x[m] = hi[i];
          x[m + step] = lo[i];
        }
      }
    } else if constexpr (NB % 4 == 0) {
#pragma unroll
      for (int k0 = 0; k0 < NB; k0 += 4) {
        uint64_t a[4], v[4], w[4], r[4], hi[4], lo[4];
#pragma unroll
        for (int i = 0; i < 4; i++) {
          const int k = k0 + i, m = (k / step) * 2 * step + (k % step);
          const uint32_t p = j + ((uint32_t)(m & (step - 1)) << log_sub);
          w[i] = tw[p << (tw_shift + (LOGR - 1 - s))];
          v[i] = x[m + step];
          a[i] = x[m];
        }
        gl::mul_n<4>(v, w, r);
        gl::canon_n<4>(r);
        gl::add_n<4>(a, r, hi);
        gl::sub_n<4>(a, r, lo);
#pragma unroll
        for (int i = 0; i < 4; i++) {
          const int k = k0 + i, m = (k / step) * 2 * step + (k % step);
          x[m] = hi[i];
          x[m + step] = lo[i];
        }
        if constexpr (LOGR >= 4) __builtin_amdgcn_sched_barrier(0);
      }
    } else {
#pragma unroll
      for (int m = 0; m < R; m++) {
        if (m & step) continue;
        const uint32_t p = j + ((uint32_t)(m & (step - 1)) << log_sub);
        const uint64_t a = x[m];
        const uint64_t t = (J0 && (m & (step - 1)) == 0) ? gl::canon(x[m + step])
                                                         : gl::mulc(x[m + step], tw[p << (tw_shift + (LOGR - 1 - s))]);
        x[m] = gl::add(a, t);
        x[m + step] = gl::sub(a, t);
      }
    }
  }
}

template <int LOGR, bool DIF>
__device__ __forceinline__ void lds_pass(uint64_t* buf, uint32_t log_blk, uint32_t span_log,
                                         const uint64_t* __restrict__ tw) {
  constexpr int R = 1 << LOGR;
  const uint32_t log_sub = span_log - LOGR, sub_mask = (1u << log_sub) - 1;
  const uint32_t n_q = 1u << (log_blk - LOGR);
  for (uint32_t q = threadIdx.x; q < n_q; q += blockDim.x) {
    const uint32_t j = q & sub_mask, blk = q >> log_sub;
    const uint32_t base = (blk << span_log) + j;
    uint64_t x[R];
#pragma unroll
    for (int m = 0; m < R; m++) x[m] = buf[base + ((uint32_t)m << log_sub)];
    if (DIF) dif_butterflies<LOGR>(x, tw, j, log_sub, log_blk - span_log);
    else dit_butterflies<LOGR>(x, tw, j, log_sub, log_blk - span_log);
#pragma unroll
    for (int m = 0; m < R; m++) buf[base + ((uint32_t)m << log_sub)] = x[m];
  }
}

struct LdsNttArgs {
  const uint64_t* in;
  uint64_t in_stride;
  uint64_t* out;
  uint64_t out_stride;
  uint64_t out_coset_stride;
  const uint64_t* tw;
  const uint64_t* scale;
  uint64_t out_scalar;
  uint32_t log_blk;
  uint32_t log_n_total;
};

template <bool DIF>
__global__ void __launch_bounds__(1024) ntt_lds_kernel(LdsNttArgs a) {
  if (gridDim.x * gridDim.y * gridDim.z <= 64) __builtin_amdgcn_s_setprio(3);
  extern __shared__ uint64_t buf[];
  const uint32_t n = 1u << a.log_blk;
  const uint64_t off = (uint64_t)blockIdx.x << a.log_blk;
  const uint64_t* src = a.in + blockIdx.y * a.in_stride + off;
  uint64_t* dst = a.out + blockIdx.y * a.out_stride + blockIdx.z * a.out_coset_stride + off;
  if (!DIF && a.scale) {
    const uint64_t* sc = a.scale + ((uint64_t)blockIdx.z << a.log_n_total) + off;
    for (uint32_t i = threadIdx.x; i < n; i += blockDim.x) buf[i] = gl::mulc(src[i], sc[i]);
  } else {
    for (uint32_t i = threadIdx.x; i < n; i += blockDim.x) buf[i] = src[i];
  }
  __syncthreads();
  const uint32_t rem = a.log_blk % 3;
  if (DIF) {
    uint32_t span = a.log_blk;
    for (; span >= 3 && span > rem; span -= 3) {
      lds_pass<3, true>(buf, a.log_blk, span, a.tw);
      __syncthreads();
    }
    if (rem == 1) lds_pass<1, true>(buf, a.log_blk, 1, a.tw);
    else if (rem == 2) lds_pass<2, true>(buf, a.log_blk, 2, a.tw);
    if (rem) __syncthreads();
  } else {
    if (rem == 1) lds_pass<1, false>(buf, a.log_blk, 1, a.tw);
    else if (rem == 2) lds_pass<2, false>(buf, a.log_blk, 2, a.tw);
    if (rem) __syncthreads();
    for (uint32_t span = rem + 3; span <= a.log_blk; span += 3) {
      lds_pass<3, false>(buf, a.log_blk, span, a.tw);
      __syncthreads();
    }
  }
  if (DIF && a.out_scalar != 1) {
    for (uint32_t i = threadIdx.x; i < n; i += blockDim.x) dst[i] = gl::mulc(buf[i], a.out_scalar);
  } else {
    for (uint32_t i = threadIdx.x; i < n; i += blockDim.x) dst[i] = gl::canon(buf[i]);
  }
}

template <int L>
__device__ __forceinline__ uint32_t swz(uint32_t i) {
  uint32_t x;
  if (L == 14) x = (((i >> 6) & 7u) << 2) ^ ((i >> 9) & 31u);
  else if (L == 13) x = (((i >> 5) & 15u) << 1) ^ ((i >> 9) & 15u);
  else x = (((i >> 8) & 1u) << 4) ^ ((i >> 7) & 1u) ^ (((i >> 9) & 7u) << 1);
  return i ^ x;
}
__device__ __forceinline__ uint32_t insert4(uint32_t t, uint32_t m, uint32_t b) {
  return ((t >> b) << (b + 4)) | (m << b) | (t & ((1u << b) - 1));
}
template <int R, int SH, bool CONTIG, bool DIF>
__device__ __forceinline__ void sub_butterflies(uint64_t (&x)[16], const uint64_t* __restrict__ tw, uint32_t j,
                                                uint32_t j_step_log, uint32_t log_sub, uint32_t tw_shift) {
  constexpr int G = 16 >> R;
#pragma unroll
  for (int g = 0; g < G; g++) {
    uint64_t y[1 << R];
#pragma unroll
    for (int u = 0; u < (1 << R); u++) y[u] = CONTIG ? x[(g << R) + u] : x[g + (u << SH)];
    const uint32_t jj = CONTIG ? 0u : j + ((uint32_t)g << j_step_log);
    if (DIF) dif_butterflies<R, CONTIG>(y, tw, jj, log_sub, tw_shift);
    else dit_butterflies<R, CONTIG>(y, tw, jj, log_sub, tw_shift);
#pragma unroll
    for (int u = 0; u < (1 << R); u++) {
      if (CONTIG) x[(g << R) + u] = y[u];
      else x[g + (u << SH)] = y[u];
    }
  }
}

struct Ntt16Args {
  const uint64_t* in;
  uint64_t in_stride;
  uint64_t* out;
  uint64_t out_stride, out_coset_stride;
  const uint64_t* tw;
  const uint64_t* scale;
  uint64_t out_scalar;
  uint32_t log_n_total, n_cosets, n_units;
  const uint64_t* tw_top;
};


template <int L, int F>
__global__ void __launch_bounds__((1 << L) / 16) ntt16_dif_kernel(Ntt16Args a) {
  if (gridDim.x * gridDim.y * gridDim.z <= 64) __builtin_amdgcn_s_setprio(3);
  extern __shared__ uint64_t buf[];
  constexpr uint32_t T = (1u << L) / 16;
  constexpr int RT = (L % 4 == 0) ? 4 : (L % 4);
  const uint32_t t = threadIdx.x;
  const uint64_t* src;
  uint64_t* dst;
  uint64_t x[16];
  if (F) {
    const uint32_t id = blockIdx.x, k = id >> 3, h = k & 1, unit = (k >> 1) * 8 + (id & 7);
    if (unit >= a.n_units) return;
    const uint32_t log_bpc = a.log_n_total - (L + 1);
    const uint32_t col = unit >> log_bpc, blk = unit & ((1u << log_bpc) - 1);
    const uint64_t off = (uint64_t)blk << (L + 1);
    src = a.in + col * a.in_stride + off;
    dst = a.out + col * a.out_stride + off + ((uint64_t)h << L);
#pragma unroll
    for (int m0 = 0; m0 < 16; m0 += 4) {
      uint64_t lo[4], hi[4], r[4];
#pragma unroll
      for (int i = 0; i < 4; i++) {
        lo[i] = src[(m0 + i) * T + t];
        hi[i] = src[(m0 + i) * T + t + (1u << L)];
      }
      gl::canon_n<4>(hi);
      if (h == 0) {
        gl::add_n<4>(lo, hi, r);
      } else {
        uint64_t d[4], w[4];
        gl::sub_n<4>(lo, hi, d);
#pragma unroll
        for (int i = 0; i < 4; i++) w[i] = a.tw_top[(m0 + i) * T + t];
        gl::mul_n<4>(d, w, r);
      }
#pragma unroll
      for (int i = 0; i < 4; i++) x[m0 + i] = r[i];
    }
  } else {
    const uint64_t off = (uint64_t)blockIdx.x << L;
    src = a.in + blockIdx.y * a.in_stride + off;
    dst = a.out + blockIdx.y * a.out_stride + off;
#pragma unroll
    for (int m = 0; m < 16; m++) x[m] = src[m * T + t];
  }
  dif_butterflies<4>(x, a.tw, t, L - 4, 0);
#pragma unroll
  for (int m = 0; m < 16; m++) buf[swz<L>(m * T + t)] = x[m];
  __syncthreads();
#pragma unroll
  for (int b = L - 8; b > 0; b -= 4) {
#pragma unroll
    for (int m = 0; m < 16; m++) x[m] = buf[swz<L>(insert4(t, m, b))];
    dif_butterflies<4>(x, a.tw, t & ((1u << b) - 1), b, L - (b + 4));
#pragma unroll
    for (int m = 0; m < 16; m++) buf[swz<L>(insert4(t, m, b))] = x[m];
    __syncthreads();
  }
  const uint32_t base = gl::bitrev(t, L - 4) << 4;
#pragma unroll
  for (int m = 0; m < 16; m++) x[m] = buf[swz<L>(base | m)];
  sub_butterflies<RT, 0, true, true>(x, a.tw, 0, 0, 0, L - RT);
#pragma unroll
  for (int m = 0; m < 16; m++) buf[swz<L>(base | m)] = x[m];
  __syncthreads();
  if (a.out_scalar != 1) {
#pragma unroll
    for (int m0 = 0; m0 < 16; m0 += 4) {
      uint64_t v[4], w[4], r[4];
#pragma unroll
      for (int i = 0; i < 4; i++) {
        v[i] = buf[swz<L>((m0 + i) * T + t)];
        w[i] = a.out_scalar;
      }
      gl::mul_n<4>(v, w, r);
      gl::canon_n<4>(r);
#pragma unroll
      for (int i = 0; i < 4; i++) dst[(m0 + i) * T + t] = r[i];
    }
  } else {
#pragma unroll
    for (int m0 = 0; m0 < 16; m0 += 4) {
      uint64_t v[4];
#pragma unroll
      for (int i = 0; i < 4; i++) v[i] = buf[swz<L>((m0 + i) * T + t)];
      gl::canon_n<4>(v);
#pragma unroll
      for (int i = 0; i < 4; i++) dst[(m0 + i) * T + t] = v[i];
    }
  }
}

template <int L, int F>
__global__ void __launch_bounds__((1 << L) / 16) __attribute__((amdgpu_waves_per_eu(4, 8))) ntt16_dit_kernel(Ntt16Args a) {
  if (gridDim.x <= 64) __builtin_amdgcn_s_setprio(3);
  extern __shared__ uint64_t buf[];
  constexpr uint32_t T = (1u << L) / 16;
  constexpr int RT = (L % 4 == 0) ? 4 : (L % 4);
  const uint32_t id = blockIdx.x, k = id >> 3;
  const uint32_t per = a.n_cosets << F;
  const uint32_t ch = k % per, coset = ch >> F, h = F ? (ch & 1) : 0, unit = (k / per) * 8 + (id & 7);
  if (unit >= a.n_units) return;
  const uint32_t log_bpc = a.log_n_total - (L + F);
  const uint32_t col = unit >> log_bpc, blk = unit & ((1u << log_bpc) - 1);
  const uint32_t t = threadIdx.x;
  const uint64_t off = (uint64_t)blk << (L + F);
  const uint64_t* src = a.in + col * a.in_stride + off;
  const uint64_t* tw = a.tw;
  uint64_t x[16];
  const uint32_t base = gl::bitrev(t, L - 4) << 4;
  if (F) {
    const ulonglong2* src2 = reinterpret_cast<const ulonglong2*>(src);
    const ulonglong2* sc2 = a.scale ? reinterpret_cast<const ulonglong2*>(a.scale + ((uint64_t)coset << a.log_n_total) + off) : nullptr;
    constexpr uint32_t BR4[16] = {0, 8, 4, 12, 2, 10, 6, 14, 1, 9, 5, 13, 3, 11, 7, 15};
#pragma unroll
    for (int m0 = 0; m0 < 16; m0 += 4) {
      uint64_t c0[4], c1[4], r[4];
#pragma unroll
      for (int i = 0; i < 4; i++) {
        const ulonglong2 c = src2[(m0 + i) * T + t];
        c0[i] = c.x;
        c1[i] = c.y;
      }
      if (sc2) {
        uint64_t s0[4], s1[4], p0[4], p1[4];
#pragma unroll
        for (int i = 0; i < 4; i++) {
          const ulonglong2 sc = sc2[(m0 + i) * T + t];
          s0[i] = sc.x;
          s1[i] = sc.y;
        }
        gl::mul_n<4>(c0, s0, p0);
        gl::mul_n<4>(c1, s1, p1);
        gl::canon_n<4>(p1);
#pragma unroll
        for (int i = 0; i < 4; i++) { c0[i] = p0[i]; c1[i] = p1[i]; }
      } else {
        gl::canon_n<4>(c1);
      }
      if (h == 0) {
        gl::add_n<4>(c0, c1, r);
      } else {
        uint64_t d[4], w[4];
        gl::sub_n<4>(c0, c1, d);
#pragma unroll
        for (int i = 0; i < 4; i++) w[i] = a.tw_top[base | BR4[m0 + i]];
        gl::mul_n<4>(d, w, r);
      }
#pragma unroll
      for (int i = 0; i < 4; i++) buf[swz<L>((m0 + i) * T + t)] = r[i];
    }
  } else if (a.scale) {
    const uint64_t* sc = a.scale + ((uint64_t)coset << a.log_n_total) + off;
#pragma unroll
    for (int m0 = 0; m0 < 16; m0 += 4) {
      uint64_t v[4], w[4], r[4];
#pragma unroll
      for (int i = 0; i < 4; i++) {
        v[i] = src[(m0 + i) * T + t];
        w[i] = sc[(m0 + i) * T + t];
      }
      gl::mul_n<4>(v, w, r);
#pragma unroll
      for (int i = 0; i < 4; i++) buf[swz<L>((m0 + i) * T + t)] = r[i];
    }
  } else {
#pragma unroll
    for (int m = 0; m < 16; m++) buf[swz<L>(m * T + t)] = src[m * T + t];
  }
  __syncthreads();
#pragma unroll
  for (int m = 0; m < 16; m++) x[m] = buf[swz<L>(base | m)];
  dit_butterflies<4, true>(x, tw, 0, 0, L - 4);
#pragma unroll
  for (int m = 0; m < 16; m++) buf[swz<L>(base | m)] = x[m];
  __syncthreads();
#pragma unroll
  for (int b = 4; b + 4 <= L - RT; b += 4) {
#pragma unroll
    for (int m = 0; m < 16; m++) x[m] = buf[swz<L>(insert4(t, m, b))];
    dit_butterflies<4>(x, tw, t & ((1u << b) - 1), b, L - (b + 4));
#pragma unroll
    for (int m = 0; m < 16; m++) buf[swz<L>(insert4(t, m, b))] = x[m];
    __syncthreads();
  }
  uint32_t t2 = t;
  asm volatile("" : "+v"(t2));
#pragma unroll
  for (int m = 0; m < 16; m++) x[m] = buf[swz<L>(m * T + t2)];
  sub_butterflies<RT, 4 - RT, false, false>(x, tw, t2, L - 4, L - RT, 0);
  uint64_t* dst = a.out + col * a.out_stride + coset * a.out_coset_stride + off;
#pragma unroll
  for (int m0 = 0; m0 < 16; m0 += 4) {
    uint64_t v[4] = {x[m0], x[m0 + 1], x[m0 + 2], x[m0 + 3]};
    gl::canon_n<4>(v);
#pragma unroll
    for (int i = 0; i < 4; i++) {
      if (F) dst[2 * ((m0 + i) * T + t2) + h] = v[i];
      else dst[(m0 + i) * T + t2] = v[i];
    }
  }
}

template <int L>
__global__ void __launch_bounds__((1 << L) / 16) __attribute__((amdgpu_waves_per_eu(4, 4)))
ntt16_dit_persist_kernel(Ntt16Args a, uint32_t n_items) {
  extern __shared__ uint64_t buf[];
  constexpr uint32_t T = (1u << L) / 16;
  constexpr int RT = (L % 4 == 0) ? 4 : (L % 4);
  const uint32_t t = threadIdx.x;
  const uint32_t log_bpc = a.log_n_total - L;
  const uint64_t* tw = a.tw;
  auto source_of = [&](uint32_t id) -> const uint64_t* {
    const uint32_t k = id >> 3, unit = (k / a.n_cosets) * 8 + (id & 7);
    if (id >= n_items || unit >= a.n_units) return nullptr;
    const uint32_t col = unit >> log_bpc, blk = unit & ((1u << log_bpc) - 1);
    return a.in + col * a.in_stride + ((uint64_t)blk << L);
  };
  uint64_t xn[16];
  {
    const uint64_t* s0 = source_of(blockIdx.x);
    if (s0) {
#pragma unroll
      for (int m = 0; m < 16; m++) xn[m] = s0[m * T + t];
    }
  }
  for (uint32_t id = blockIdx.x; id < n_items; id += gridDim.x) {
    const uint32_t k = id >> 3, coset = k % a.n_cosets, unit = (k / a.n_cosets) * 8 + (id & 7);
    const uint64_t* next_src = source_of(id + gridDim.x);
    uint32_t ta = t, tb = t, tc = t;
    asm volatile("" : "+v"(ta));
    if (unit >= a.n_units) {
      if (next_src) {
#pragma unroll
        for (int m = 0; m < 16; m++) xn[m] = next_src[m * T + t];
      }
      continue;
    }
    const uint32_t col = unit >> log_bpc, blk = unit & ((1u << log_bpc) - 1);
    const uint64_t off = (uint64_t)blk << L;
    if (a.scale) {
      const uint64_t* sc = a.scale + ((uint64_t)coset << a.log_n_total) + off;
#pragma unroll
      for (int m0 = 0; m0 < 16; m0 += 4) {
        uint64_t v[4], w[4], r[4];
#pragma unroll
        for (int i = 0; i < 4; i++) {
          v[i] = xn[m0 + i];
          w[i] = sc[(m0 + i) * T + ta];
        }
        gl::mul_n<4>(v, w, r);
#pragma unroll
        for (int i = 0; i < 4; i++) buf[swz<L>((m0 + i) * T + ta)] = r[i];
      }
    } else {
#pragma unroll
      for (int m = 0; m < 16; m++) buf[swz<L>(m * T + ta)] = xn[m];
    }
    __syncthreads();
    asm volatile("" : "+v"(tb));
    const uint32_t base = gl::bitrev(tb, L - 4) << 4;
    uint64_t x[16];
#pragma unroll
    for (int m = 0; m < 16; m++) x[m] = buf[swz<L>(base | m)];
    dit_butterflies<4, true>(x, tw, 0, 0, L - 4);
#pragma unroll
    for (int m = 0; m < 16; m++) buf[swz<L>(base | m)] = x[m];
    __syncthreads();
#pragma unroll
    for (int b = 4; b + 4 <= L - RT; b += 4) {
      asm volatile("" : "+v"(tc));
#pragma unroll
      for (int m = 0; m < 16; m++) x[m] = buf[swz<L>(insert4(tc, m, b))];
      dit_butterflies<4>(x, tw, tc & ((1u << b) - 1), b, L - (b + 4));
#pragma unroll
      for (int m = 0; m < 16; m++) buf[swz<L>(insert4(tc, m, b))] = x[m];
      __syncthreads();
    }
    uint32_t t2 = t;
    asm volatile("" : "+v"(t2));
    if (next_src) {
#pragma unroll
      for (int m = 0; m < 16; m++) xn[m] = next_src[m * T + t2];
    }
#pragma unroll
    for (int m = 0; m < 16; m++) x[m] = buf[swz<L>(m * T + t2)];
    sub_butterflies<RT, 4 - RT, false, false>(x, tw, t2, L - 4, L - RT, 0);
    uint64_t* dst = a.out + col * a.out_stride + coset * a.out_coset_stride + off;
#pragma unroll
    for (int m0 = 0; m0 < 16; m0 += 4) {
      uint64_t v[4] = {x[m0], x[m0 + 1], x[m0 + 2], x[m0 + 3]};
      gl::canon_n<4>(v);
#pragma unroll
      for (int i = 0; i < 4; i++) dst[(m0 + i) * T + t2] = v[i];
    }
  }
}

#include "ntt_mx.cuh"

template <int LOGR, bool DIF>
__global__ void __launch_bounds__(256)
ntt_global_pass_kernel(const uint64_t* in, uint64_t in_stride, uint64_t* out, uint64_t out_stride,
                       uint64_t coset_stride, uint32_t log_n, uint32_t span_log,
                       const uint64_t* __restrict__ tw) {
  constexpr int R = 1 << LOGR;
  const uint32_t log_sub = span_log - LOGR;
  const uint32_t q = blockIdx.x * blockDim.x + threadIdx.x;
  if (q >= (1u << (log_n - LOGR))) return;
  const uint32_t j = q & ((1u << log_sub) - 1), blk = q >> log_sub;
  const uint64_t base = ((uint64_t)blk << span_log) + j;
  const uint64_t* src = in + blockIdx.y * in_stride + blockIdx.z * coset_stride + base;
  uint64_t* dst = out + blockIdx.y * out_stride + blockIdx.z * coset_stride + base;
  uint64_t x[R];
#pragma unroll
  for (int m = 0; m < R; m++) x[m] = src[(uint64_t)m << log_sub];
  if (DIF) dif_butterflies<LOGR>(x, tw, j, log_sub, log_n - span_log);
  else dit_butterflies<LOGR>(x, tw, j, log_sub, log_n - span_log);
  if constexpr (R % 4 == 0) {
#pragma unroll
    for (int m0 = 0; m0 < R; m0 += 4) {
      uint64_t v[4] = {x[m0], x[m0 + 1], x[m0 + 2], x[m0 + 3]};
      gl::canon_n<4>(v);
#pragma unroll
      for (int i = 0; i < 4; i++) dst[(uint64_t)(m0 + i) << log_sub] = v[i];
    }
  } else {
#pragma unroll
    for (int m = 0; m < R; m++) dst[(uint64_t)m << log_sub] = gl::canon(x[m]);
  }
}


template <int A, bool DIF>
__global__ void __launch_bounds__(1 << A)
ntt_tile_kernel(const uint64_t* in, uint64_t in_stride, uint64_t* out, uint64_t out_stride, uint64_t coset_stride,
                uint32_t log_n, uint32_t span_log, const uint64_t* __restrict__ tw) {
  constexpr int R = 1 << A, B = A - 4, R1 = 1 << B, G = 16 / R1;
  __shared__ uint64_t tile[R * 16];
  const uint32_t log_s = span_log - A;
  const uint32_t tiles_per_blk = 1u << (log_s - 4);
  const uint32_t blk = blockIdx.x / tiles_per_blk, s0 = (blockIdx.x % tiles_per_blk) << 4;
  const uint32_t s = threadIdx.x & 15, hi = threadIdx.x >> 4;
  const uint64_t base = ((uint64_t)blk << span_log) + s0 + s;
  const uint64_t* src = in + blockIdx.y * in_stride + blockIdx.z * coset_stride + base;
  uint64_t* dst = out + blockIdx.y * out_stride + blockIdx.z * coset_stride + base;
  const uint32_t j16 = (hi << log_s) + s0 + s;
  uint64_t x[16];
  if (DIF) {
#pragma unroll
    for (int m = 0; m < 16; m++) x[m] = src[(uint64_t)(hi + m * (R / 16)) << log_s];
    dif_butterflies<4>(x, tw, j16, span_log - 4, log_n - span_log);
#pragma unroll
    for (int m = 0; m < 16; m++) tile[(hi + m * (R / 16)) * 16 + s] = x[m];
    __syncthreads();
#pragma unroll
    for (int m = 0; m < 16; m++) x[m] = tile[(hi * 16 + m) * 16 + s];
#pragma unroll
    for (int g = 0; g < G; g++) {
      uint64_t y[R1];
#pragma unroll
      for (int u = 0; u < R1; u++) y[u] = x[g * R1 + u];
      dif_butterflies<B>(y, tw, s0 + s, log_s, log_n - span_log + 4);
#pragma unroll
      for (int u = 0; u < R1; u++) x[g * R1 + u] = y[u];
    }
#pragma unroll
    for (int m0 = 0; m0 < 16; m0 += 4) {
      uint64_t v[4] = {x[m0], x[m0 + 1], x[m0 + 2], x[m0 + 3]};
      gl::canon_n<4>(v);
#pragma unroll
      for (int i = 0; i < 4; i++) dst[(uint64_t)(hi * 16 + m0 + i) << log_s] = v[i];
    }
  } else {
#pragma unroll
    for (int m = 0; m < 16; m++) x[m] = src[(uint64_t)(hi * 16 + m) << log_s];
#pragma unroll
    for (int g = 0; g < G; g++) {
      uint64_t y[R1];
#pragma unroll
      for (int u = 0; u < R1; u++) y[u] = x[g * R1 + u];
      dit_butterflies<B>(y, tw, s0 + s, log_s, log_n - span_log + 4);
#pragma unroll
      for (int u = 0; u < R1; u++) x[g * R1 + u] = y[u];
    }
#pragma unroll
    for (int m = 0; m < 16; m++) tile[(hi * 16 + m) * 16 + s] = x[m];
    __syncthreads();
#pragma unroll
    for (int m = 0; m < 16; m++) x[m] = tile[(hi + m * (R / 16)) * 16 + s];
    dit_butterflies<4>(x, tw, j16, span_log - 4, log_n - span_log);
#pragma unroll
    for (int m0 = 0; m0 < 16; m0 += 4) {
      uint64_t v[4] = {x[m0], x[m0 + 1], x[m0 + 2], x[m0 + 3]};
      gl::canon_n<4>(v);
#pragma unroll
      for (int i = 0; i < 4; i++) dst[(uint64_t)(hi + (m0 + i) * (R / 16)) << log_s] = v[i];
    }
  }
}

__global__ void twiddle_table_kernel(uint64_t* out, uint32_t count, uint64_t w) {
  uint32_t e = blockIdx.x * blockDim.x + threadIdx.x;
  if (e < count) out[e] = gl::pow(w, e);
}
__global__ void coset_scale_table_kernel(uint64_t* out, uint32_t log_n, uint32_t rate_bits, uint64_t w_m,
                                         int inverse) {
  uint32_t pos = blockIdx.x * blockDim.x + threadIdx.x;
  if (pos >= (1u << log_n)) return;
  uint32_t t = blockIdx.y;
  uint64_t g = gl::mulc(gl::GENERATOR, gl::pow(w_m, t));
  if (inverse) g = gl::inv(g);
  out[((uint64_t)t << log_n) + pos] = gl::pow(g, gl::bitrev(pos, log_n));
}
__global__ void bitrev_permute_kernel(uint64_t* cols, uint64_t stride, uint32_t log_n) {
  uint32_t i = blockIdx.x * blockDim.x + threadIdx.x;
  if (i >= (1u << log_n)) return;
  uint32_t j = gl::bitrev(i, log_n);
  if (i < j) {
    uint64_t* c = cols + blockIdx.y * stride;
    uint64_t a = c[i], b = c[j];
    c[i] = b;
    c[j] = a;
  }
}

struct TableKey {
  int dev, kind;
  uint32_t log_n, rate_bits;
  bool operator<(const TableKey& o) const {
    return std::tie(dev, kind, log_n, rate_bits) < std::tie(o.dev, o.kind, o.log_n, o.rate_bits);
  }
};
std::mutex g_table_mu;
std::map<TableKey, uint64_t*> g_tables;

}

namespace bpg {

int get_table(int kind, uint32_t log_n, uint32_t rate_bits, const uint64_t** out) {
  int dev = 0;
  BPG_HIP(hipGetDevice(&dev));
  std::lock_guard<std::mutex> lk(g_table_mu);
  TableKey key{dev, kind, log_n, kind >= 2 ? rate_bits : 0};
  auto it = g_tables.find(key);
  if (it != g_tables.end()) {
    *out = it->second;
    return BP_OK;
  }
  uint64_t* d = nullptr;
  if (kind >= 2) {
    uint64_t count = (uint64_t)1 << (log_n + rate_bits);
    BPG_HIP(hipMalloc(&d, count * 8));
    dim3 grid(ceil_div((uint64_t)1 << log_n, 256), 1u << rate_bits);
    coset_scale_table_kernel<<<grid, 256, 0, 0>>>(d, log_n, rate_bits, gl::root(log_n + rate_bits), kind == 3);
  } else {
    uint32_t count = log_n ? (1u << (log_n - 1)) : 1;
    BPG_HIP(hipMalloc(&d, (uint64_t)count * 8));
    uint64_t w = gl::root(log_n);
    if (kind == 1) w = gl::inv(w);
    twiddle_table_kernel<<<ceil_div(count, 256), 256, 0, 0>>>(d, count, w);
  }
  BPG_LAUNCH_CHECK();
  BPG_HIP(hipStreamSynchronize(0));
  g_tables[key] = d;
  *out = d;
  return BP_OK;
}

bool device_loaded();
static std::atomic<int> g_ntt_mx{3};
static bool use_ntt_mx(uint32_t log_blk, bool dit) {
  const int m = g_ntt_mx.load(std::memory_order_relaxed);
  if (m == 3) return log_blk == 13 && !device_loaded();
  if (m == 4) return !dit && log_blk <= 13;
  if (m == 5) return dit && log_blk <= 13;
  return m == 2 || (m == 1 && log_blk <= 13);
}
static std::mutex g_mx_mu;
static std::map<std::tuple<int, int, int>, mxn::Tables*> g_mx_tabs;
static std::atomic<int> g_mx_wg_per_cu{0};
static uint32_t mx_grid(uint32_t items, uint32_t log_blk) {
  static const int cus = [] {
    int dev = 0, n = 256;
    if (hipGetDevice(&dev) == hipSuccess) (void)hipDeviceGetAttribute(&n, hipDeviceAttributeMultiprocessorCount, dev);
    return n > 0 ? n : 256;
  }();
  int per = g_mx_wg_per_cu.load(std::memory_order_relaxed);
  if (per <= 0) per = log_blk == 12 ? 2 : 1;
  const uint32_t resident = ((uint32_t)cus * per + 7) / 8 * 8;
  return items < resident ? items : resident;
}
static int get_mx_tables(int kind, bool inverse, const mxn::Tables** out) {
  int dev = 0;
  BPG_HIP(hipGetDevice(&dev));
  std::lock_guard<std::mutex> lk(g_mx_mu);
  const auto key = std::make_tuple(dev, kind, inverse ? 1 : 0);
  auto it = g_mx_tabs.find(key);
  if (it != g_mx_tabs.end()) {
    *out = it->second;
    return BP_OK;
  }
  auto host = std::make_unique<mxn::Tables>();
  mxn::build_tables(*host, kind, inverse);
  mxn::Tables* d = nullptr;
  BPG_HIP(hipMalloc(&d, sizeof(mxn::Tables)));
  BPG_HIP(hipMemcpy(d, host.get(), sizeof(mxn::Tables), hipMemcpyHostToDevice));
  g_mx_tabs[key] = d;
  *out = d;
  return BP_OK;
}

struct NttPlan {
  uint32_t log_blk;
  uint32_t tile_bits;
  uint32_t n_reg;
  uint32_t reg_bits[4];
};
static NttPlan plan_ntt(uint32_t log_n) {
  NttPlan p{};
  if (log_n <= LOG_BLK_MAX) { p.log_blk = log_n; return p; }
  if (log_n <= 17) { p.log_blk = log_n <= 16 ? 12 : 13; p.n_reg = 1; p.reg_bits[0] = log_n - p.log_blk; return p; }
  if (log_n <= 20) { p.log_blk = 12; p.tile_bits = log_n - 12; return p; }
  if (log_n <= 22) { p.log_blk = log_n - 8; p.tile_bits = 8; return p; }
  p.log_blk = 14; p.tile_bits = 8;
  uint32_t left = log_n - 22;
  p.n_reg = (left + 3) / 4;
  for (uint32_t i = 0; i < p.n_reg; i++) {
    const uint32_t k = (left + (p.n_reg - i) - 1) / (p.n_reg - i);
    p.reg_bits[i] = k;
    left -= k;
  }
  return p;
}
static uint32_t pick_log_blk(uint32_t log_n) { return plan_ntt(log_n).log_blk; }

static std::atomic<int> g_ntt_persist{0};
static std::atomic<int> g_ntt_persist_wgs{256};
static std::atomic<int> g_ntt_split{0};
static bool use_split(uint32_t log_blk, uint64_t workgroups, const void* src, const void* dst, bool dit) {
  const int mode = g_ntt_split.load(std::memory_order_relaxed);
  if (mode == 1 || log_blk < 13 || src == dst) return false;
  if (mode == 2) return true;
  if (dit) return mode == 3 && log_blk == 13 && workgroups < 512;
  return log_blk == 14 || workgroups < 512;
}

static uint32_t lds_threads(uint32_t log_blk) {
  uint32_t t = log_blk >= 3 ? (1u << (log_blk - 3)) : 1;
  return t < 64 ? 64 : (t > 1024 ? 1024 : t);
}

template <bool DIF>
static int launch_global_passes(const uint64_t* in, uint64_t in_stride, uint64_t* out, uint64_t out_stride,
                                uint64_t coset_stride, uint32_t n_cols, uint32_t n_cosets, uint32_t log_n,
                                uint32_t log_blk, const uint64_t* tw, hipStream_t st) {
  const NttPlan p = plan_ntt(log_n);
  uint32_t spans[8], bits[8], tiled[8], cnt = 0;
  uint32_t span = log_n;
  for (uint32_t i = 0; i < p.n_reg; i++) { spans[cnt] = span; bits[cnt] = p.reg_bits[i]; tiled[cnt] = 0; cnt++; span -= p.reg_bits[i]; }
  if (p.tile_bits) { spans[cnt] = span; bits[cnt] = p.tile_bits; tiled[cnt] = 1; cnt++; span -= p.tile_bits; }
  if (span != log_blk || log_blk != p.log_blk) return fail(BP_ERR_DEVICE, "NTT plan mismatch (log_n=%u)", log_n);
  for (uint32_t idx = 0; idx < cnt; idx++) {
    const uint32_t i = DIF ? idx : cnt - 1 - idx;
    const uint64_t* src = (idx == 0) ? in : out;
    const uint64_t src_stride = (idx == 0) ? in_stride : out_stride;
    if (tiled[i]) {
      const dim3 grid(1u << (log_n - bits[i] - 4), n_cols, n_cosets);
      switch (bits[i]) {
        case 6: ntt_tile_kernel<6, DIF><<<grid, 64, 0, st>>>(src, src_stride, out, out_stride, coset_stride, log_n, spans[i], tw); break;
        case 7: ntt_tile_kernel<7, DIF><<<grid, 128, 0, st>>>(src, src_stride, out, out_stride, coset_stride, log_n, spans[i], tw); break;
        default: ntt_tile_kernel<8, DIF><<<grid, 256, 0, st>>>(src, src_stride, out, out_stride, coset_stride, log_n, spans[i], tw); break;
      }
    } else {
      const dim3 grid(ceil_div((uint64_t)1 << (log_n - bits[i]), 256), n_cols, n_cosets);
      switch (bits[i]) {
        case 1: ntt_global_pass_kernel<1, DIF><<<grid, 256, 0, st>>>(src, src_stride, out, out_stride, coset_stride, log_n, spans[i], tw); break;
        case 2: ntt_global_pass_kernel<2, DIF><<<grid, 256, 0, st>>>(src, src_stride, out, out_stride, coset_stride, log_n, spans[i], tw); break;
        case 3: ntt_global_pass_kernel<3, DIF><<<grid, 256, 0, st>>>(src, src_stride, out, out_stride, coset_stride, log_n, spans[i], tw); break;
        case 4: ntt_global_pass_kernel<4, DIF><<<grid, 256, 0, st>>>(src, src_stride, out, out_stride, coset_stride, log_n, spans[i], tw); break;
        default: return fail(BP_ERR_DEVICE, "NTT plan asks for a %u-stage register pass", bits[i]);
      }
    }
    BPG_LAUNCH_CHECK();
  }
  return BP_OK;
}

int intt_nat2br(const uint64_t* in, uint64_t in_stride, uint64_t* out, uint64_t out_stride, uint32_t log_n,
                uint32_t n_cols, bool inverse, hipStream_t st) {
  if (n_cols == 0) return BP_OK;
  const uint32_t log_blk = pick_log_blk(log_n);
  const uint64_t *tw_n = nullptr, *tw_b = nullptr;
  int rc;
  if ((rc = get_table(inverse ? 1 : 0, log_blk, 0, &tw_b))) return rc;
  const uint64_t* src = in;
  uint64_t src_stride = in_stride;
  if (log_n > LOG_BLK_MAX) {
    if ((rc = get_table(inverse ? 1 : 0, log_n, 0, &tw_n))) return rc;
    if ((rc = launch_global_passes<true>(in, in_stride, out, out_stride, 0, n_cols, 1, log_n, log_blk, tw_n, st))) return rc;
    src = out;
    src_stride = out_stride;
  }
  if (log_blk >= 12) {
    Ntt16Args b{};
    b.in = src; b.in_stride = src_stride; b.out = out; b.out_stride = out_stride; b.out_coset_stride = 0;
    b.tw = tw_b; b.scale = nullptr; b.out_scalar = inverse ? gl::inv((uint64_t)1 << log_n) : 1;
    b.log_n_total = log_n; b.n_cosets = 1; b.n_units = 0;
    KernelTimer kt(PROF_INTT_DIF, st, 16.0 * (double)n_cols * (double)((uint64_t)1 << log_n));
    if (use_ntt_mx(log_blk, false)) {
      const mxn::Tables* tab = nullptr;
      if ((rc = get_mx_tables(0, inverse, &tab))) return rc;
      b.n_units = n_cols << (log_n - log_blk);
      const uint32_t g = mx_grid(b.n_units, log_blk);
      if (log_blk == 12) mxn::ntt_mx_dif_kernel<0><<<g, 256, (8u << 12) + 4 * mxn::C_LDS_WORDS, st>>>(b, tab);
      else if (log_blk == 13) mxn::ntt_mx_dif_kernel<1><<<g, 512, (8u << 13) + 4 * mxn::C_LDS_WORDS, st>>>(b, tab);
      else mxn::ntt_mx_dif_kernel<2><<<g, 512, (8u << 14) + 4 * mxn::C_LDS_WORDS, st>>>(b, tab);
    } else if (use_split(log_blk, (uint64_t)n_cols << (log_n - log_blk), src, out, false)) {
      if ((rc = get_table(inverse ? 1 : 0, log_blk - 1, 0, &b.tw))) return rc;
      b.tw_top = tw_b;
      b.n_units = n_cols << (log_n - log_blk);
      const dim3 grid1((b.n_units + 7) / 8 * 8 * 2);
      if (log_blk == 14) ntt16_dif_kernel<13, 1><<<grid1, 512, 8u << 13, st>>>(b);
      else ntt16_dif_kernel<12, 1><<<grid1, 256, 8u << 12, st>>>(b);
    } else {
      const dim3 grid16(1u << (log_n - log_blk), n_cols);
      if (log_blk == 12) ntt16_dif_kernel<12, 0><<<grid16, 256, 8u << 12, st>>>(b);
      else if (log_blk == 13) ntt16_dif_kernel<13, 0><<<grid16, 512, 8u << 13, st>>>(b);
      else ntt16_dif_kernel<14, 0><<<grid16, 1024, 8u << 14, st>>>(b);
    }
    BPG_LAUNCH_CHECK();
    return BP_OK;
  }
  LdsNttArgs a{};
  a.in = src; a.in_stride = src_stride; a.out = out; a.out_stride = out_stride; a.out_coset_stride = 0;
  a.tw = tw_b; a.scale = nullptr;
  a.out_scalar = inverse ? gl::inv((uint64_t)1 << log_n) : 1;
  a.log_blk = log_blk; a.log_n_total = log_n;
  dim3 grid(1u << (log_n - log_blk), n_cols, 1);
  size_t lds = (size_t)8 << log_blk;
  {
    KernelTimer kt(PROF_INTT_DIF, st, 16.0 * (double)n_cols * (double)((uint64_t)1 << log_n));
    ntt_lds_kernel<true><<<grid, lds_threads(log_blk), lds, st>>>(a);
  }
  BPG_LAUNCH_CHECK();
  return BP_OK;
}

int ntt_br2nat(const uint64_t* in, uint64_t in_stride, uint64_t* out, uint64_t out_stride, uint64_t coset_stride,
               uint32_t log_n, uint32_t n_cols, uint32_t n_cosets, const uint64_t* scale, bool inverse,
               hipStream_t st) {
  if (n_cols == 0) return BP_OK;
  const uint32_t log_blk = pick_log_blk(log_n);
  const uint64_t *tw_n = nullptr, *tw_b = nullptr;
  int rc;
  if ((rc = get_table(inverse ? 1 : 0, log_blk, 0, &tw_b))) return rc;
  if (log_blk >= 12) {
    Ntt16Args b{};
    b.in = in; b.in_stride = in_stride; b.out = out; b.out_stride = out_stride; b.out_coset_stride = coset_stride;
    b.tw = tw_b; b.scale = scale; b.out_scalar = 1; b.log_n_total = log_n; b.n_cosets = n_cosets;
    b.n_units = n_cols << (log_n - log_blk);
    {
      KernelTimer kt(PROF_LDE_DIT, st, 8.0 * (double)n_cols * (double)((uint64_t)1 << log_n) * (1.0 + n_cosets), true);
      if (use_ntt_mx(log_blk, true)) {
        const mxn::Tables* tab = nullptr;
        if ((rc = get_mx_tables(1, inverse, &tab))) return rc;
        const uint32_t g = mx_grid((b.n_units + 7) / 8 * 8 * n_cosets, log_blk);
        if (log_blk == 12) BPG_LAUNCH_TIMED(kt, mxn::ntt_mx_dit_kernel<0>, g, 256, (8u << 12) + 4 * mxn::C_LDS_WORDS, st, b, tab);
        else if (log_blk == 13) BPG_LAUNCH_TIMED(kt, mxn::ntt_mx_dit_kernel<1>, g, 512, (8u << 13) + 4 * mxn::C_LDS_WORDS, st, b, tab);
        else BPG_LAUNCH_TIMED(kt, mxn::ntt_mx_dit_kernel<2>, g, 512, (8u << 14) + 4 * mxn::C_LDS_WORDS, st, b, tab);
      } else if (use_split(log_blk, (uint64_t)b.n_units * n_cosets, in, out, true)) {
        if ((rc = get_table(inverse ? 1 : 0, log_blk - 1, 0, &b.tw))) return rc;
        b.tw_top = tw_b;
        const dim3 grid1((b.n_units + 7) / 8 * 8 * n_cosets * 2);
        if (log_blk == 14) BPG_LAUNCH_TIMED(kt, HIP_KERNEL_NAME(ntt16_dit_kernel<13, 1>), grid1, 512, 8u << 13, st, b);
        else BPG_LAUNCH_TIMED(kt, HIP_KERNEL_NAME(ntt16_dit_kernel<12, 1>), grid1, 256, 8u << 12, st, b);
      } else {
        const dim3 grid16((b.n_units + 7) / 8 * 8 * n_cosets);
        if (log_blk == 12) BPG_LAUNCH_TIMED(kt, HIP_KERNEL_NAME(ntt16_dit_kernel<12, 0>), grid16, 256, 8u << 12, st, b);
        else if (log_blk == 13) BPG_LAUNCH_TIMED(kt, HIP_KERNEL_NAME(ntt16_dit_kernel<13, 0>), grid16, 512, 8u << 13, st, b);
        else {
          const uint32_t items = grid16.x, group = 8 * n_cosets;
          const uint32_t resident = std::max<uint32_t>(group, (uint32_t)g_ntt_persist_wgs.load(std::memory_order_relaxed) / group * group);
          if (g_ntt_persist.load(std::memory_order_relaxed) && items > resident && in != out)
            BPG_LAUNCH_TIMED(kt, HIP_KERNEL_NAME(ntt16_dit_persist_kernel<14>), dim3(resident), 1024, 8u << 14, st, b, items);
          else
            BPG_LAUNCH_TIMED(kt, HIP_KERNEL_NAME(ntt16_dit_kernel<14, 0>), grid16, 1024, 8u << 14, st, b);
        }
      }
    }
    BPG_LAUNCH_CHECK();
  } else {
  LdsNttArgs a{};
  a.in = in; a.in_stride = in_stride; a.out = out; a.out_stride = out_stride; a.out_coset_stride = coset_stride;
  a.tw = tw_b; a.scale = scale; a.out_scalar = 1; a.log_blk = log_blk; a.log_n_total = log_n;
  dim3 grid(1u << (log_n - log_blk), n_cols, n_cosets);
  size_t lds = (size_t)8 << log_blk;
  {
    KernelTimer kt(PROF_LDE_DIT, st, 8.0 * (double)n_cols * (double)((uint64_t)1 << log_n) * (1.0 + n_cosets), true);
    BPG_LAUNCH_TIMED(kt, ntt_lds_kernel<false>, grid, lds_threads(log_blk), lds, st, a);
  }
  BPG_LAUNCH_CHECK();
  }
  if (log_n > LOG_BLK_MAX) {
    if ((rc = get_table(inverse ? 1 : 0, log_n, 0, &tw_n))) return rc;
    if ((rc = launch_global_passes<false>(out, out_stride, out, out_stride, coset_stride, n_cols, n_cosets, log_n,
                                          log_blk, tw_n, st)))
      return rc;
  }
  return BP_OK;
}

int bitrev_permute(uint64_t* cols, uint64_t stride, uint32_t log_n, uint32_t n_cols, hipStream_t st) {
  dim3 grid(ceil_div((uint64_t)1 << log_n, 256), n_cols);
  bitrev_permute_kernel<<<grid, 256, 0, st>>>(cols, stride, log_n);
  BPG_LAUNCH_CHECK();
  return BP_OK;
}

static int init_ntt_kernels_once() {
  BPG_HIP(hipFuncSetAttribute(reinterpret_cast<const void*>(&ntt_lds_kernel<true>),
                              hipFuncAttributeMaxDynamicSharedMemorySize, 8 << LOG_BLK_MAX));
  BPG_HIP(hipFuncSetAttribute(reinterpret_cast<const void*>(&ntt_lds_kernel<false>),
                              hipFuncAttributeMaxDynamicSharedMemorySize, 8 << LOG_BLK_MAX));
  BPG_HIP(hipFuncSetAttribute(reinterpret_cast<const void*>(&ntt16_dif_kernel<14, 0>),
                              hipFuncAttributeMaxDynamicSharedMemorySize, 8 << 14));
  BPG_HIP(hipFuncSetAttribute(reinterpret_cast<const void*>(&ntt16_dit_kernel<14, 0>),
                              hipFuncAttributeMaxDynamicSharedMemorySize, 8 << 14));
  BPG_HIP(hipFuncSetAttribute(reinterpret_cast<const void*>(&ntt16_dit_persist_kernel<14>),
                              hipFuncAttributeMaxDynamicSharedMemorySize, 8 << 14));
  BPG_HIP(hipFuncSetAttribute(reinterpret_cast<const void*>(&ntt16_dif_kernel<13, 0>),
                              hipFuncAttributeMaxDynamicSharedMemorySize, 8 << 13));
  BPG_HIP(hipFuncSetAttribute(reinterpret_cast<const void*>(&ntt16_dit_kernel<13, 0>),
                              hipFuncAttributeMaxDynamicSharedMemorySize, 8 << 13));
  BPG_HIP(hipFuncSetAttribute(reinterpret_cast<const void*>(&mxn::ntt_mx_dif_kernel<1>),
                              hipFuncAttributeMaxDynamicSharedMemorySize, (8 << 13) + 4 * mxn::C_LDS_WORDS));
  BPG_HIP(hipFuncSetAttribute(reinterpret_cast<const void*>(&mxn::ntt_mx_dif_kernel<2>),
                              hipFuncAttributeMaxDynamicSharedMemorySize, (8 << 14) + 4 * mxn::C_LDS_WORDS));
  BPG_HIP(hipFuncSetAttribute(reinterpret_cast<const void*>(&mxn::ntt_mx_dit_kernel<1>),
                              hipFuncAttributeMaxDynamicSharedMemorySize, (8 << 13) + 4 * mxn::C_LDS_WORDS));
  BPG_HIP(hipFuncSetAttribute(reinterpret_cast<const void*>(&mxn::ntt_mx_dit_kernel<2>),
// ... 128 lines not shown
```

proof_protocol_decoder_amd/csrc/stark_kernels.hip:

```cpp
#include "common.hpp"
#include "gl.hpp"
#include "poseidon.cuh"
#include "poseidon_mx.cuh"
#include "stark_kernels.hpp"
#include "quotient_dev.cuh"
#include "air_program.hpp"

namespace {

using gl::Ext;
using namespace bpg::k5;

__device__ __forceinline__ uint64_t splitmix64(uint64_t x) {
  uint64_t z = x + 0x9E3779B97F4A7C15ULL;
  z = (z ^ (z >> 30)) * 0xBF58476D1CE4E5B9ULL;
  z = (z ^ (z >> 27)) * 0x94D049BB133111EBULL;
  return z ^ (z >> 31);
}
__device__ __forceinline__ uint64_t rnd(uint64_t seed, uint64_t col, uint64_t row) {
  return gl::canon(splitmix64(seed ^ (col << 32) ^ row));
}
__device__ __forceinline__ uint64_t pow_e(uint64_t t, uint32_t e) {
  return e == 3 ? gl::mulc(gl::mulc(t, t), t) : t;
}
// ... 993 lines not shown
      e[m][0] = a.values[2 * (base[m] + o0) + comp];
      e[m][1] = a.values[2 * (base[m] + o1) + comp];
    }
    poseidon::mx::permute<NS>(e, c);
  }
#pragma unroll
  for (int m = 0; m < NS; m++) {
    const uint64_t id = id0 + 16 * m;
    if (id < n_leaves) {
      const uint32_t t = (uint32_t)(id >> log_q), m0 = (uint32_t)(id & ((1u << log_q) - 1));
      const uint64_t leaf = gl::bitrev((uint32_t)(t + ((uint64_t)m0 << a.rate_bits)), log_q + a.rate_bits);
      a.digests[leaf * 4 + c.kb] = gl::canon(e[m][0]);
    }
  }
}
__global__ void __launch_bounds__(256) fri_fold_kernel(bpg::BatchOf<bpg::FriLayerArgs> batch) {
  if (gridDim.x * gridDim.y * gridDim.z <= 64) __builtin_amdgcn_s_setprio(3);
  const bpg::FriLayerArgs& a = batch.a[blockIdx.z];
  const uint32_t log_q = a.log_nl - a.arity_bits;
  const uint64_t n_out = (uint64_t)1 << (log_q + a.rate_bits);
  const uint64_t id = blockIdx.x * (uint64_t)blockDim.x + threadIdx.x;
  if (id >= n_out) return;
  const uint32_t t = (uint32_t)(id >> log_q), m0 = (uint32_t)(id & ((1u << log_q) - 1));
  const uint64_t base = ((uint64_t)t << a.log_nl) + m0;
  const uint64_t x_inv = gl::mulc(a.g_t_inv[t], root_pow(a.tw_nl_inv, a.log_nl, m0));
  uint64_t c0[16], c1[16];
#pragma unroll
  for (int j = 0; j < 16; j++) {
    const uint64_t p = base + ((uint64_t)j << log_q);
    c0[j] = a.values[2 * p];
    c1[j] = a.values[2 * p + 1];
  }
#pragma unroll
  for (int s = 0; s < 4; s++) {
    const int half = 8 >> s;
#pragma unroll
    for (int k0 = 0; k0 < 8; k0 += 2) {
      uint64_t d[4], w[4], r[4];
      int mm[2];
#pragma unroll
      for (int i = 0; i < 2; i++) {
        const int k = k0 + i, m = (k / half) * 2 * half + (k % half);
        mm[i] = m;
        const uint64_t wv = a.wa_inv_pow[(m & (half - 1)) << s];
        const uint64_t x0 = c0[m], x1 = c1[m], y0 = c0[m + half], y1 = c1[m + half];
        c0[m] = gl::addc(x0, y0);
        c1[m] = gl::addc(x1, y1);
        d[2 * i] = gl::subc(x0, y0);
        d[2 * i + 1] = gl::subc(x1, y1);
        w[2 * i] = wv;
        w[2 * i + 1] = wv;
      }
      if (half == 1) {
#pragma unroll
        for (int i = 0; i < 4; i++) r[i] = d[i];
      } else {
        gl::mul_n<4>(d, w, r);
#pragma unroll
        for (int i = 0; i < 4; i++) r[i] = gl::canon(r[i]);
        __builtin_amdgcn_sched_barrier(0);
      }
#pragma unroll
      for (int i = 0; i < 2; i++) {
        c0[mm[i] + half] = r[2 * i];
        c1[mm[i] + half] = r[2 * i + 1];
      }
    }
  }
  const Ext bx = gl::scale(a.beta, x_inv);
  Ext acc = gl::ext(0);
#pragma unroll
  for (int i = 15; i >= 0; i--) {
    const int slot = ((i & 1) << 3) | ((i & 2) << 1) | ((i & 4) >> 1) | ((i & 8) >> 3);
    acc = gl::add(gl::mul(acc, bx), Ext{c0[slot], c1[slot]});
  }
  acc = gl::scale(acc, a.arity_inv);
  a.out[2 * id] = acc.c0;
  a.out[2 * id + 1] = acc.c1;
}

__global__ void __launch_bounds__(256) pow_grind_kernel(bpg::BatchOf<bpg::PowArgs> batch, unsigned long long* result) {
  const bpg::PowArgs& a = batch.a[blockIdx.z];
  result += blockIdx.z;
  if (__hip_atomic_load(result, __ATOMIC_RELAXED, __HIP_MEMORY_SCOPE_AGENT) < a.base) return;
  const uint64_t cand = a.base + blockIdx.x * (uint64_t)blockDim.x + threadIdx.x;
  uint64_t s[12];
#pragma unroll
  for (int k = 0; k < 12; k++) s[k] = a.state[k];
  s[a.pos] = cand;
  poseidon::permute(s);
  if ((gl::canon(s[7]) >> (64 - a.bits)) == 0) atomicMin(result, (unsigned long long)cand);
}
template <int GR>
__global__ void __launch_bounds__(256) __attribute__((amdgpu_waves_per_eu(3)))
pow_grind_mx_kernel(bpg::BatchOf<bpg::PowArgs> batch, unsigned long long* result, const uint32_t* __restrict__ gtab) {
  const bpg::PowArgs& a = batch.a[blockIdx.z];
  result += blockIdx.z;
  if (__hip_atomic_load(result, __ATOMIC_RELAXED, __HIP_MEMORY_SCOPE_AGENT) < a.base) return;
  constexpr int NG = GR ? GR : 2;
  __shared__ __attribute__((aligned(16))) uint32_t cin[GR ? poseidon::mx::CIN_GROUPED_WORDS<NG> : poseidon::mx::CIN_WORDS];
  __shared__ __attribute__((aligned(16))) uint32_t gt[GR ? poseidon::mx::grp::TABLE_WORDS<NG> : 4];
  if constexpr (GR != 0) {
    poseidon::mx::build_cin_grouped<NG>(cin);
    poseidon::mx::grp::load_tables<NG>(gt, gtab);
  } else {
    poseidon::mx::build_cin(cin);
  }
  __syncthreads();
  const poseidon::mx::Ctx c = poseidon::mx::make_ctx(cin);
  const uint64_t cand0 = a.base + ((uint64_t)blockIdx.x * 4 + (threadIdx.x >> 6)) * 64 + (threadIdx.x & 15);
  uint64_t e[4][3];
#pragma unroll
  for (int s = 0; s < 3; s++) {
    uint64_t w = a.state[4 * s];
#pragma unroll
    for (int q = 1; q < 4; q++) w = c.kb == (uint32_t)q ? a.state[4 * s + q] : w;
    const bool mine = c.kb + 4 * s == a.pos;
#pragma unroll
    for (int m = 0; m < 4; m++) e[m][s] = mine ? cand0 + 16 * m : w;
  }
  if constexpr (GR != 0) poseidon::mx::permute_grouped<NG>(e, c, gt, gtab);
  else poseidon::mx::permute<4>(e, c);
  if (c.kb == 3) {
#pragma unroll
    for (int m = 0; m < 4; m++)
      if ((gl::canon(e[m][1]) >> (64 - a.bits)) == 0) atomicMin(result, (unsigned long long)(cand0 + 16 * m));
  }
}

__global__ void __launch_bounds__(256) query_initial_kernel(bpg::QueryArgs a) {
  if (gridDim.x * gridDim.y * gridDim.z <= 64) __builtin_amdgcn_s_setprio(3);
  const uint32_t b = blockIdx.x / a.n_queries, q = blockIdx.x % a.n_queries, o = blockIdx.y;
  const uint64_t x = a.x_index[blockIdx.x];
  const bpg::QueryOracle& orc = a.proof[b].oracle[o];
  const uint32_t log_rows = a.log_n + a.rate_bits;
  const uint32_t i = gl::bitrev((uint32_t)x, log_rows);
  const uint64_t pos = ((uint64_t)(i & ((1u << a.rate_bits) - 1)) << a.log_n) + (i >> a.rate_bits);
  uint64_t* out = a.proof[b].out;
  if (o == 0 && threadIdx.x == 0) out[(uint64_t)q * a.query_words] = x;
  uint64_t* w = out + (uint64_t)q * a.query_words + orc.out_offset;
  for (uint32_t c = threadIdx.x; c < orc.n_cols; c += blockDim.x) w[c] = orc.lde[(uint64_t)c * orc.stride + pos];
  w += orc.n_cols;
  const uint32_t depth = log_rows - a.cap_height;
  for (uint32_t k = threadIdx.x; k < depth * 4; k += blockDim.x) {
    const uint32_t lvl = k >> 2;
    const uint64_t off = ((uint64_t)2 << log_rows) - ((uint64_t)2 << (log_rows - lvl));
    w[k] = orc.digests[(off + ((x >> lvl) ^ 1)) * 4 + (k & 3)];
  }
  if (q == 0 && o == a.leaf_oracle && a.proof[b].first_leaf && threadIdx.x < 4) a.proof[b].first_leaf[threadIdx.x] = orc.digests[x * 4 + threadIdx.x];
}
__global__ void __launch_bounds__(64) query_layers_kernel(bpg::QueryLayerArgs a) {
  if (gridDim.x * gridDim.y * gridDim.z <= 64) __builtin_amdgcn_s_setprio(3);
  const uint32_t b = blockIdx.x / a.n_queries, q = blockIdx.x % a.n_queries, l = blockIdx.y;
  const bpg::QueryLayer& L = a.proof[b].layer[l];
  const uint32_t arity = 1u << a.arity_bits;
  const uint64_t leaf = a.x_index[blockIdx.x] >> (a.arity_bits * (l + 1));
  const uint32_t log_q = L.log_nl - a.arity_bits, log_leaves = log_q + a.rate_bits;
  const uint32_t c = gl::bitrev((uint32_t)leaf, log_leaves);
  const uint32_t t = c & ((1u << a.rate_bits) - 1), m0 = c >> a.rate_bits;
  const uint64_t base = ((uint64_t)t << L.log_nl) + m0;
  uint64_t* w = a.proof[b].out + (uint64_t)q * a.query_words + L.out_offset;
  for (uint32_t k = threadIdx.x; k < 2 * arity; k += blockDim.x) {
    const uint32_t jj = gl::bitrev(k >> 1, a.arity_bits);
    w[k] = L.values[2 * (base + ((uint64_t)jj << log_q)) + (k & 1)];
  }
  w += 2 * arity;
  const uint32_t depth = log_leaves - a.cap_height;
  for (uint32_t k = threadIdx.x; k < depth * 4; k += blockDim.x) {
    const uint32_t lvl = k >> 2;
    const uint64_t off = ((uint64_t)2 << log_leaves) - ((uint64_t)2 << (log_leaves - lvl));
    w[k] = L.digests[(off + ((leaf >> lvl) ^ 1)) * 4 + (k & 3)];
  }
}

}

namespace bpg {

int launch_synth_constants(uint64_t* d_out, uint32_t log_n, uint32_t n_const, uint64_t seed, hipStream_t st) {
  uint64_t total = (uint64_t)n_const << log_n;
  if (!total) return BP_OK;
// ... 303 lines not shown
```

proof_protocol_decoder_amd/ops.py:

```python
import ctypes as C

import numpy as np
import torch

from ._lib import StarkCfg, check, lib, take_buffer

NTT_FWD_BR2NAT, NTT_INV_NAT2BR, NTT_FWD_NAT, NTT_INV_NAT = 0, 1, 2, 3


def _stream():
    return torch.cuda.current_stream().cuda_stream


def _require_cuda(t):
    if not t.is_cuda:
        raise ValueError("bpg ops need device tensors (there is no CPU fallback)")
    if t.dtype != torch.int64 or not t.is_contiguous():
        raise ValueError("bpg ops need contiguous int64 tensors holding u64 bit patterns")


def ntt_batch_(cols, direction):
    _require_cuda(cols)
    n_cols, n = cols.shape
    check(lib().bp_ntt_batch(cols.data_ptr(), n.bit_length() - 1, n_cols, n, direction, _stream()))
    return cols


def intt_batch(values, out=None):
    import ctypes as C
    _require_cuda(values)
    n_cols, n = values.shape
    out = torch.empty_like(values) if out is None else out
    L = lib()
    L.bp_intt_batch.argtypes = [C.c_void_p, C.c_uint64, C.c_void_p, C.c_uint64, C.c_uint32, C.c_uint32, C.c_void_p]
    check(L.bp_intt_batch(values.data_ptr(), n, out.data_ptr(), n, n.bit_length() - 1, n_cols, _stream()))
    return out


def lde_batch(inp, rate_bits, from_coeffs=False):
    _require_cuda(inp)
    n_cols, n = inp.shape
    coeffs = torch.empty_like(inp)
    lde = torch.empty((n_cols, n << rate_bits), dtype=torch.int64, device=inp.device)
    check(lib().bp_lde_batch(inp.data_ptr(), n, coeffs.data_ptr(), n, lde.data_ptr(), n << rate_bits,
                             n.bit_length() - 1, rate_bits, n_cols, int(from_coeffs), _stream()))
    return coeffs, lde


def poseidon_perm_batch_(states):
    _require_cuda(states)
    check(lib().bp_poseidon_perm_batch(states.data_ptr(), states.numel() // 12, _stream()))
    return states


def field_ops(a, b):
    _require_cuda(a)
    _require_cuda(b)
    n = a.numel()
    out = torch.empty((15, n), dtype=torch.int64, device=a.device)
    check(lib().bp_debug_field_ops(a.data_ptr(), b.data_ptr(), out.data_ptr(), n, _stream()))
    return out


AIR_SYNTHETIC, AIR_KECCAK_F = 0, 1
KECCAK_COLS = 2431
LOGIC_COLS = 524
MEMORY_COLS = 45
ARITHMETIC_COLS = 309
BYTE_PACKING_COLS = 299
KECCAK_SPONGE_COLS = 2414
ARITHMETIC_MUL_COLS = 1217


def air_describe(air_id, n_cols=0, n_const=0, deg_pow=1):
    from ._lib import AirDesc
    d = AirDesc()
    check(lib().bp_air_describe(air_id, n_cols, n_const, deg_pow, C.byref(d)))
    return d


def air_register(words):
    words = np.ascontiguousarray(words, dtype=np.uint64)
    air_id = C.c_uint32()
    check(lib().bp_air_register(words.ctypes.data, words.size, C.byref(air_id)))
    return air_id.value


def air_unregister(air_id):
    check(lib().bp_air_unregister(air_id))


def air_program_digest(air_id):
    out = C.create_string_buffer(32)
    check(lib().bp_air_program_digest(air_id, out))
    return out.raw


def _table_trace(name, n_cols, in_shape, log_n, seed, inputs, device):
    out = torch.empty((n_cols, 1 << log_n), dtype=torch.int64, device=device)
    if inputs is not None:
        _require_cuda(inputs)
        assert inputs.shape == in_shape
    check(getattr(lib(), "bp_%s_trace" % name)(inputs.data_ptr() if inputs is not None else None, seed, log_n, out.data_ptr(),
                                               _stream()))
    return out


def logic_trace(log_n, seed=0, inputs=None, device="cuda"):
    return _table_trace("logic", LOGIC_COLS, (1 << log_n, 9), log_n, seed, inputs, device)


def memory_trace(log_n, seed=0, inputs=None, device="cuda"):
    return _table_trace("memory", MEMORY_COLS, (1 << log_n, 11), log_n, seed, inputs, device)


def arithmetic_trace(log_n, seed=0, inputs=None, device="cuda"):
    return _table_trace("arithmetic", ARITHMETIC_COLS, (1 << log_n, 9), log_n, seed, inputs, device)


def byte_packing_trace(log_n, seed=0, inputs=None, device="cuda"):
    return _table_trace("byte_packing", BYTE_PACKING_COLS, (1 << log_n, 6), log_n, seed, inputs, device)


def keccak_sponge_trace(log_n, seed=0, inputs=None, device="cuda"):
    return _table_trace("keccak_sponge", KECCAK_SPONGE_COLS, (1 << log_n, 44), log_n, seed, inputs, device)


def arithmetic_mul_trace(log_n, seed=0, inputs=None, device="cuda"):
    return _table_trace("arithmetic_mul", ARITHMETIC_MUL_COLS, (1 << log_n, 9), log_n, seed, inputs, device)


def keccak_trace(log_n, seed=0, inputs=None, device="cuda"):
    return _table_trace("keccak", KECCAK_COLS, (((1 << log_n) + 23) // 24, 25), log_n, seed, inputs, device)


def quotient_eval(cfg, trace_lde, aux_lde, const_lde, ctl, alphas, air_id=AIR_SYNTHETIC):
    _require_cuda(trace_lde)
    _require_cuda(aux_lde)
    if const_lde is not None:
        _require_cuda(const_lde)
    rows = trace_lde.shape[1]
    scratch = torch.empty(int(lib().bp_quotient_scratch_words(air_id, C.byref(cfg))), dtype=torch.int64,
                          device=trace_lde.device)
# ... 165 lines not shown
```

Baseline: 33.85.

## Use shift-based power-of-two twiddles in radix-16 NTT passes with per-layer tables

In the Goldilocks field the 16th roots of unity are powers of two (2^12 steps), so the new code replaces the generic 64-bit multiplies inside each radix-16 butterfly with shift-and-reduce sequences. It adds dif16/dit16 kernels that read a precomputed per-layer twiddle table for the inter-group twiddles, and removes the old J0 grouped-multiply path. The 16-point fast path only applies to the forward LDE and the inverse INTT kernels. The PoW grind kernels also get an earlier per-block exit once a smaller nonce has been found, and a debug mul_pow2 entry point is added for testing. The cost is more complex NTT code, a new table allocation, and a correctness risk in the hand-written carry logic.

```diff
diff --git a/include/bpg.h b/include/bpg.h
--- a/include/bpg.h
+++ b/include/bpg.h
@@ -38,6 +38,7 @@
 int bp_debug_copy_u64(const uint64_t* d_in, uint64_t* d_out, uint64_t n, void* stream);
 
 int bp_debug_field_ops(const uint64_t* d_a, const uint64_t* d_b, uint64_t* d_out, uint64_t n, void* stream);
+int bp_debug_mul_pow2(const uint64_t* d_a, uint64_t* d_out, uint64_t n, void* stream);
 
 void bp_tune_quad_threshold(uint64_t n_perms);
 void bp_tune_merkle_fused(int mode);
diff --git a/proof_protocol_decoder_amd/_lib.py b/proof_protocol_decoder_amd/_lib.py
--- a/proof_protocol_decoder_amd/_lib.py
+++ b/proof_protocol_decoder_amd/_lib.py
@@ -68,6 +68,7 @@
     L.bp_lde_batch.argtypes = [vp, u64, vp, u64, vp, u64, u32, u32, u32, i, vp]
     L.bp_poseidon_perm_batch.argtypes = [vp, u64, vp]
     L.bp_debug_field_ops.argtypes = [vp, vp, vp, u64, vp]
+    L.bp_debug_mul_pow2.argtypes = [vp, vp, u64, vp]
     L.bp_quotient_scratch_words.argtypes = [u32, C.POINTER(StarkCfg)]
     L.bp_quotient_scratch_words.restype = u64
     L.bp_quotient_eval.argtypes = [u32, C.POINTER(StarkCfg), vp, vp, vp, C.POINTER(u64), C.POINTER(u64), vp, vp, vp]
diff --git a/proof_protocol_decoder_amd/csrc/gl.hpp b/proof_protocol_decoder_amd/csrc/gl.hpp
--- a/proof_protocol_decoder_amd/csrc/gl.hpp
+++ b/proof_protocol_decoder_amd/csrc/gl.hpp
@@ -23,6 +23,11 @@
 __device__ __forceinline__ uint64_t mad_eps_co(uint32_t a, uint64_t c, mask& co) {
   uint64_t d;
   asm("v_mad_u64_u32 %0, %1, %2, -1, %3" : "=v"(d), "=s"(co) : "v"(a), "v"(c));
+  return d;
+}
+__device__ __forceinline__ uint64_t mul_eps(uint32_t a) {
+  uint64_t d;
+  asm("v_mad_u64_u32 %0, vcc, %1, -1, 0" : "=v"(d) : "v"(a) : "vcc");
   return d;
 }
 __device__ __forceinline__ uint32_t add_co(uint32_t a, uint32_t b, mask& co) {
@@ -230,6 +235,134 @@
   for (int i = 0; i < N; i++) a[i] = cc::mk64(lo[i], hi[i]);
 }
 #endif
+GL_HD uint64_t mul_pow2_portable(uint64_t x, unsigned S) {
+  if (S < 64) return reduce128(x << S, S ? x >> (64 - S) : 0);
+  const unsigned s = S - 64;
+  const uint64_t lo = x << s, hi = s ? x >> (64 - s) : 0;
+  return sub(reduce128(0, lo), hi << 32);
+}
+#if defined(__HIP__)
+__device__ __forceinline__ void shl96(uint64_t x, int s, uint32_t& l0, uint32_t& l1, uint32_t& l2) {
+  const uint32_t x0 = (uint32_t)x, x1 = (uint32_t)(x >> 32);
+  l0 = x0 << s;
+  l1 = (x1 << s) | (x0 >> (32 - s));
+  l2 = x1 >> (32 - s);
+}
+__device__ __forceinline__ uint64_t mul_pow2_lo(uint64_t x, int s) {
+  uint32_t l0, l1, l2;
+  shl96(x, s, l0, l1, l2);
+  cc::mask c3, b3, cx;
+  const uint64_t V = cc::mad_eps_co(l2, cc::mk64(l0, l1), c3);
+  const uint32_t t0 = cc::subb0_co((uint32_t)V, c3, b3);
+  const uint32_t t1 = cc::addc0_co((uint32_t)(V >> 32), c3 & ~b3, cx);
+  return cc::mk64(t0, t1);
+}
+__device__ __forceinline__ uint64_t mul_2p32(uint64_t y) {
+  cc::mask c3, b3, cx;
+  const uint64_t V = cc::mul_eps((uint32_t)(y >> 32));
+  const uint32_t h = cc::add_co((uint32_t)(V >> 32), (uint32_t)y, c3);
+  const uint32_t t0 = cc::subb0_co((uint32_t)V, c3, b3);
+  const uint32_t t1 = cc::addc0_co(h, c3 & ~b3, cx);
+  return cc::mk64(t0, t1);
+}
+__device__ __forceinline__ uint64_t mul_pow2_hi(uint64_t x, int s) {
+  uint32_t l0, l1, l2;
+  shl96(x, s, l0, l1, l2);
+  cc::mask bw, bw2, b3, cx;
+  const uint64_t D = cc::mul_eps(l0);
+  const uint32_t t0 = cc::sub_co((uint32_t)D, l1, bw);
+  const uint32_t t1 = cc::subb_co((uint32_t)(D >> 32), l2, bw, bw2);
+  const uint32_t r0 = cc::addc0_co(t0, bw2, b3);
+  const uint32_t r1 = cc::subb0_co(t1, bw2 & ~b3, cx);
+  return cc::mk64(r0, r1);
+}
+template <int N>
+__device__ __forceinline__ void mul_pow2_lo_n(const uint64_t (&a)[N], const int (&s)[N], uint64_t (&r)[N]) {
+  static_assert(N == 3 || N == 4, "groups of 3 or 4");
+  uint32_t l2[N], t0[N], t1[N];
+  uint64_t P[N];
+  cc::mask c3[N], b3[N];
+#pragma unroll
+  for (int i = 0; i < N; i++) {
+    uint32_t l0, l1;
+    shl96(a[i], s[i], l0, l1, l2[i]);
+    P[i] = cc::mk64(l0, l1);
+  }
+  cc::mad_eps_co(P, c3, l2);
+#pragma unroll
+  for (int i = 0; i < N; i++) { t0[i] = (uint32_t)P[i]; t1[i] = (uint32_t)(P[i] >> 32); }
+  cc::subb0_co(t0, b3, c3);
+#pragma unroll
+  for (int i = 0; i < N; i++) c3[i] &= ~b3[i];
+  cc::addc0_cv(t1, c3);
+#pragma unroll
+  for (int i = 0; i < N; i++) r[i] = cc::mk64(t0[i], t1[i]);
+}
+template <int N>
+__device__ __forceinline__ void mul_2p32_n(const uint64_t (&a)[N], uint64_t (&r)[N]) {
+  static_assert(N == 3 || N == 4, "groups of 3 or 4");
+  uint32_t y0[N], y1[N], t0[N], t1[N];
+  uint64_t V[N];
+  cc::mask c3[N], b3[N];
+#pragma unroll
+  for (int i = 0; i < N; i++) { y0[i] = (uint32_t)a[i]; y1[i] = (uint32_t)(a[i] >> 32); }
+  cc::mul_eps_o(V, y1);
+#pragma unroll
+  for (int i = 0; i < N; i++) { t0[i] = (uint32_t)V[i]; t1[i] = (uint32_t)(V[i] >> 32); }
+  cc::add_co(t1, c3, y0);
+  cc::subb0_co(t0, b3, c3);
+#pragma unroll
+  for (int i = 0; i < N; i++) c3[i] &= ~b3[i];
+  cc::addc0_cv(t1, c3);
+#pragma unroll
+  for (int i = 0; i < N; i++) r[i] = cc::mk64(t0[i], t1[i]);
+}
+template <int N>
+__device__ __forceinline__ void mul_pow2_hi_n(const uint64_t (&a)[N], const int (&s)[N], uint64_t (&r)[N]) {
+  static_assert(N == 3 || N == 4, "groups of 3 or 4");
+  uint32_t l0[N], l1[N], l2[N], t0[N], t1[N];
+  uint64_t D[N];
+  cc::mask bw[N], bw2[N], b3[N];
+#pragma unroll
+  for (int i = 0; i < N; i++) shl96(a[i], s[i], l0[i], l1[i], l2[i]);
+  cc::mul_eps_o(D, l0);
+#pragma unroll
+  for (int i = 0; i < N; i++) { t0[i] = (uint32_t)D[i]; t1[i] = (uint32_t)(D[i] >> 32); }
+  cc::sub_co(t0, bw, l1);
+  cc::subb_co(t1, bw2, l2, bw);
+  cc::addc0_co(t0, b3, bw2);
+#pragma unroll
+  for (int i = 0; i < N; i++) bw2[i] &= ~b3[i];
+  cc::subb0_cv(t1, bw2);
+#pragma unroll
+  for (int i = 0; i < N; i++) r[i] = cc::mk64(t0[i], t1[i]);
+}
+template <int S, int N>
+__device__ __forceinline__ void mul_pow2_n(const uint64_t (&a)[N], uint64_t (&r)[N]) {
+  static_assert(0 < S && S < 96 && S % 32 != 0, "2^S with 0 < S < 96, S no multiple of 32");
+  int s[N];
+#pragma unroll
+  for (int i = 0; i < N; i++) s[i] = S % 32;
+  if constexpr (S < 32) {
+    mul_pow2_lo_n<N>(a, s, r);
+  } else if constexpr (S < 64) {
+    uint64_t y[N];
+    mul_pow2_lo_n<N>(a, s, y);
+    mul_2p32_n<N>(y, r);
+  } else {
+    mul_pow2_hi_n<N>(a, s, r);
+  }
+}
+#endif
+GL_HD uint64_t mul_pow2(uint64_t x, unsigned S) {
+#if defined(__HIP_DEVICE_COMPILE__)
+  if (S < 32) return mul_pow2_lo(x, (int)S);
+  if (S < 64) return mul_2p32(mul_pow2_lo(x, (int)S - 32));
+  return mul_pow2_hi(x, (int)S - 64);
+#else
+  return mul_pow2_portable(x, S);
+#endif
+}
 #if defined(__HIP__)
 struct DotAcc {
   uint64_t p, m, q;
diff --git a/proof_protocol_decoder_amd/csrc/gl_cc.inc b/proof_protocol_decoder_amd/csrc/gl_cc.inc
--- a/proof_protocol_decoder_amd/csrc/gl_cc.inc
+++ b/proof_protocol_decoder_amd/csrc/gl_cc.inc
@@ -108,6 +108,11 @@
       : "=&v"(x[0]), "=&v"(x[1]), "=&v"(x[2]), "=&s"(co[0]), "=&s"(co[1]), "=&s"(co[2])
       : "v"(a[0]), "v"(a[1]), "v"(a[2]), "s"(ci[0]), "s"(ci[1]), "s"(ci[2]));
 }
+__device__ __forceinline__ void mul_eps_o(uint64_t (&x)[3], const uint32_t (&a)[3]) {
+  asm("v_mad_u64_u32 %0, vcc, %3, -1, 0\n\tv_mad_u64_u32 %1, vcc, %4, -1, 0\n\tv_mad_u64_u32 %2, vcc, %5, -1, 0"
+      : "=&v"(x[0]), "=&v"(x[1]), "=&v"(x[2])
+      : "v"(a[0]), "v"(a[1]), "v"(a[2]) : "vcc");
+}
 __device__ __forceinline__ void mad_co(uint64_t (&x)[4], mask (&co)[4], const uint32_t (&a)[4], const uint32_t (&b)[4]) {
   asm("v_mad_u64_u32 %0, %4, %8, %12, %0\n\tv_mad_u64_u32 %1, %5, %9, %13, %1\n\tv_mad_u64_u32 %2, %6, %10, %14, %2\n\tv_mad_u64_u32 %3, %7, %11, %15, %3"
       : "+v"(x[0]), "+v"(x[1]), "+v"(x[2]), "+v"(x[3]), "=&s"(co[0]), "=&s"(co[1]), "=&s"(co[2]), "=&s"(co[3])
@@ -218,3 +223,8 @@
       : "=&v"(x[0]), "=&v"(x[1]), "=&v"(x[2]), "=&v"(x[3]), "=&s"(co[0]), "=&s"(co[1]), "=&s"(co[2]), "=&s"(co[3])
       : "v"(a[0]), "v"(a[1]), "v"(a[2]), "v"(a[3]), "s"(ci[0]), "s"(ci[1]), "s"(ci[2]), "s"(ci[3]));
 }
+__device__ __forceinline__ void mul_eps_o(uint64_t (&x)[4], const uint32_t (&a)[4]) {
+  asm("v_mad_u64_u32 %0, vcc, %4, -1, 0\n\tv_mad_u64_u32 %1, vcc, %5, -1, 0\n\tv_mad_u64_u32 %2, vcc, %6, -1, 0\n\tv_mad_u64_u32 %3, vcc, %7, -1, 0"
+      : "=&v"(x[0]), "=&v"(x[1]), "=&v"(x[2]), "=&v"(x[3])
+      : "v"(a[0]), "v"(a[1]), "v"(a[2]), "v"(a[3]) : "vcc");
+}
diff --git a/proof_protocol_decoder_amd/csrc/hash_kernels.hip b/proof_protocol_decoder_amd/csrc/hash_kernels.hip
--- a/proof_protocol_decoder_amd/csrc/hash_kernels.hip
+++ b/proof_protocol_decoder_amd/csrc/hash_kernels.hip
@@ -433,6 +433,33 @@
   }
 }
 
+template <int K>
+__device__ __forceinline__ void mul_pow2_planes(const uint64_t (&x)[4], uint64_t* __restrict__ out, uint64_t n, uint64_t i0) {
+  uint64_t r4[4], r3[3];
+  const uint64_t x3[3] = {x[1], x[2], x[3]};
+  gl::mul_pow2_n<12 * K, 4>(x, r4);
+  __builtin_amdgcn_sched_barrier(0);
+  gl::mul_pow2_n<12 * K, 3>(x3, r3);
+  __builtin_amdgcn_sched_barrier(0);
+#pragma unroll
+  for (int k = 0; k < 4; k++) {
+    const uint64_t i = i0 + k;
+    if (i >= n) break;
+    out[(3 * (K - 1) + 0) * n + i] = gl::canon(r4[k]);
+    out[(3 * (K - 1) + 1) * n + i] = k ? gl::canon(r3[k - 1]) : gl::canon(r4[0]);
+    out[(3 * (K - 1) + 2) * n + i] = gl::canon(gl::mul_pow2(x[k], 12 * K));
+  }
+  if constexpr (K < 7) mul_pow2_planes<K + 1>(x, out, n, i0);
+}
+__global__ void __launch_bounds__(256) mul_pow2_kernel(const uint64_t* __restrict__ a, uint64_t* __restrict__ out, uint64_t n) {
+  const uint64_t i0 = (blockIdx.x * (uint64_t)blockDim.x + threadIdx.x) * 4;
+  if (i0 >= n) return;
+  uint64_t x[4];
+#pragma unroll
+  for (int k = 0; k < 4; k++) x[k] = a[i0 + k < n ? i0 + k : n - 1];
+  mul_pow2_planes<1>(x, out, n, i0);
+}
+
 __global__ void __launch_bounds__(256)
 calib_copy_u64_kernel(const uint64_t* __restrict__ in, uint64_t* __restrict__ out, uint64_t n) {
   uint64_t i = blockIdx.x * (uint64_t)blockDim.x + threadIdx.x;
@@ -709,6 +736,14 @@
   return BP_OK;
 }
 
+int bp_debug_mul_pow2(const uint64_t* d_a, uint64_t* d_out, uint64_t n, void* stream) {
+  if (!n) return BP_OK;
+  if (!d_a || !d_out) return bpg::fail(BP_ERR_INVALID_INPUT, "bp_debug_mul_pow2: null buffer");
+  mul_pow2_kernel<<<bpg::ceil_div(bpg::ceil_div(n, 4), 256), 256, 0, bpg::as_stream(stream)>>>(d_a, d_out, n);
+  BPG_LAUNCH_CHECK();
+  return BP_OK;
+}
+
 void bp_tune_merkle_fused(int mode) { bpg::g_merkle_fused.store(mode < 0 ? -1 : (mode >= 8 && mode <= 20 ? mode : (mode != 0))); }
 void bp_tune_quad_threshold(uint64_t n_perms) { bpg::g_quad_threshold.store(n_perms); }
 void bp_tune_poseidon_mx(int on) { bpg::g_poseidon_mx.store(on != 0); }
diff --git a/proof_protocol_decoder_amd/csrc/ntt.hip b/proof_protocol_decoder_amd/csrc/ntt.hip
--- a/proof_protocol_decoder_amd/csrc/ntt.hip
+++ b/proof_protocol_decoder_amd/csrc/ntt.hip
@@ -12,25 +12,6 @@
 
 constexpr uint32_t LOG_BLK_MAX = 14;
 
-template <int N>
-__device__ __forceinline__ void mul_group(uint64_t (&x)[16], const int (&idx)[4], const uint64_t (&d)[4], const uint64_t (&w)[4]) {
-  if constexpr (N == 4) {
-    uint64_t r[4];
-    gl::mul_n<4>(d, w, r);
-#pragma unroll
-    for (int i = 0; i < 4; i++) x[idx[i]] = r[i];
-  } else if constexpr (N == 3) {
-    const uint64_t d3[3] = {d[0], d[1], d[2]}, w3[3] = {w[0], w[1], w[2]};
-    uint64_t r[3];
-    gl::mul_n<3>(d3, w3, r);
-#pragma unroll
-    for (int i = 0; i < 3; i++) x[idx[i]] = r[i];
-  } else {
-#pragma unroll
-    for (int i = 0; i < N; i++) x[idx[i]] = gl::mul(d[i], w[i]);
-  }
-}
-
 template <int LOGR, bool J0 = false>
 __device__ __forceinline__ void dif_butterflies(uint64_t (&x)[1 << LOGR], const uint64_t* __restrict__ tw,
                                                 uint32_t j, uint32_t log_sub, uint32_t tw_shift) {
@@ -38,55 +19,7 @@
 #pragma unroll
   for (int s = 0; s < LOGR; s++) {
     const int half = R >> (s + 1);
-    if constexpr (NB % 4 == 0 && J0 && LOGR == 4) {
-      uint64_t dd[NB];
-#pragma unroll
-      for (int k0 = 0; k0 < NB; k0 += 4) {
-        uint64_t a[4], b[4], d[4], r[4];
-#pragma unroll
-        for (int i = 0; i < 4; i++) {
-          const int k = k0 + i, m = (k / half) * 2 * half + (k % half);
-          a[i] = x[m];
-          b[i] = x[m + half];
-        }
-        gl::canon_n<4>(b);
-        gl::add_n<4>(a, b, r);
-        gl::sub_n<4>(a, b, d);
-#pragma unroll
-        for (int i = 0; i < 4; i++) {
-          const int k = k0 + i, m = (k / half) * 2 * half + (k % half);
-          x[m] = r[i];
-          dd[k] = d[i];
-        }
-      }
-      int cnt = 0;
-      int idx[4] = {0, 0, 0, 0};
-      uint64_t dv[4] = {0, 0, 0, 0}, wv[4] = {0, 0, 0, 0};
-      uint64_t xx[16];
-#pragma unroll
-      for (int i = 0; i < 16; i++) xx[i] = x[i];
-#pragma unroll
-      for (int k = 0; k < NB; k++) {
-        const int m = (k / half) * 2 * half + (k % half), e = m & (half - 1);
-        if (e == 0) {
-          xx[m + half] = dd[k];
-        } else {
-          idx[cnt] = m + half;
-          dv[cnt] = dd[k];
-          wv[cnt] = tw[(uint32_t)e << (tw_shift + s)];
-          cnt++;
-          if (cnt == 4) {
-            mul_group<4>(xx, idx, dv, wv);
-            cnt = 0;
-          }
-        }
-      }
-      if (cnt == 3) mul_group<3>(xx, idx, dv, wv);
-      else if (cnt == 2) mul_group<2>(xx, idx, dv, wv);
-      else if (cnt == 1) mul_group<1>(xx, idx, dv, wv);
-#pragma unroll
-      for (int i = 0; i < 16; i++) x[i] = xx[i];
-    } else if constexpr (NB % 4 == 0) {
+    if constexpr (NB % 4 == 0) {
 #pragma unroll
       for (int k0 = 0; k0 < NB; k0 += 4) {
         uint64_t a[4], b[4], d[4], w[4], r[4];
@@ -137,50 +70,7 @@
 #pragma unroll
   for (int s = 0; s < LOGR; s++) {
     const int step = 1 << s;
-    if constexpr (NB % 4 == 0 && J0 && LOGR == 4) {
-      uint64_t xx[16];
-#pragma unroll
-      for (int i = 0; i < 16; i++) xx[i] = x[i];
-      int cnt = 0;
-      int idx[4] = {0, 0, 0, 0};
-      uint64_t dv[4] = {0, 0, 0, 0}, wv[4] = {0, 0, 0, 0};
-#pragma unroll
-      for (int k = 0; k < NB; k++) {
-        const int m = (k / step) * 2 * step + (k % step), e = m & (step - 1);
-        if (e != 0) {
-          idx[cnt] = m + step;
-          dv[cnt] = x[m + step];
-          wv[cnt] = tw[(uint32_t)e << (tw_shift + (LOGR - 1 - s))];
-          cnt++;
-          if (cnt == 4) {
-            mul_group<4>(xx, idx, dv, wv);
-            cnt = 0;
-          }
-        }
-      }
-      if (cnt == 3) mul_group<3>(xx, idx, dv, wv);
-      else if (cnt == 2) mul_group<2>(xx, idx, dv, wv);
-      else if (cnt == 1) mul_group<1>(xx, idx, dv, wv);
-#pragma unroll
-      for (int k0 = 0; k0 < NB; k0 += 4) {
-        uint64_t a[4], r[4], hi[4], lo[4];
-#pragma unroll
-        for (int i = 0; i < 4; i++) {
-          const int k = k0 + i, m = (k / step) * 2 * step + (k % step);
-          a[i] = xx[m];
-          r[i] = xx[m + step];
-        }
-        gl::canon_n<4>(r);
-        gl::add_n<4>(a, r, hi);
-        gl::sub_n<4>(a, r, lo);
-#pragma unroll
-        for (int i = 0; i < 4; i++) {
-          const int k = k0 + i, m = (k / step) * 2 * step + (k % step);
-          x[m] = hi[i];
-          x[m + step] = lo[i];
-        }
-      }
-    } else if constexpr (NB % 4 == 0) {
+    if constexpr (NB % 4 == 0) {
 #pragma unroll
       for (int k0 = 0; k0 < NB; k0 += 4) {
         uint64_t a[4], v[4], w[4], r[4], hi[4], lo[4];
@@ -217,6 +107,148 @@
       }
     }
   }
+}
+
+constexpr int brev4(int m) { return ((m & 1) << 3) | ((m & 2) << 1) | ((m & 4) >> 1) | ((m & 8) >> 3); }
+
+struct Pow2Plan {
+  int n_lo, n_mid, n_hi;
+  int lo_idx[8], lo_sh[8], mid_idx[8], hi_idx[8], hi_sh[8];
+};
+constexpr Pow2Plan pow2_plan(int s, bool dif) {
+  Pow2Plan p{};
+  for (int k = 0; k < 8; k++) {
+    const int h = dif ? (8 >> s) : (1 << s);
+    const int m = (k / h) * 2 * h + (k % h);
+    const int e = (m & (h - 1)) << (dif ? s : 3 - s);
+    if (e == 0) continue;
+    const int S = 12 * e;
+    if (S < 64) {
+      p.lo_idx[p.n_lo] = m + h; p.lo_sh[p.n_lo] = S % 32; p.n_lo++;
+      if (S >= 32) p.mid_idx[p.n_mid++] = m + h;
+    } else {
+      p.hi_idx[p.n_hi] = m + h; p.hi_sh[p.n_hi] = S - 64; p.n_hi++;
+    }
+  }
+  return p;
+}
+template <int STEP, int CNT, int I0 = 0>
+__device__ __forceinline__ void apply_pow2(uint64_t (&x)[16], const int (&idx)[8], const int (&sh)[8]) {
+  constexpr int LEFT = CNT - I0, N = LEFT >= 4 ? 4 : LEFT;
+  if constexpr (N >= 3) {
+    uint64_t v[N], r[N];
+    int s[N];
+#pragma unroll
+    for (int i = 0; i < N; i++) { v[i] = x[idx[I0 + i]]; s[i] = sh[I0 + i]; }
+    if constexpr (STEP == 0) gl::mul_pow2_lo_n<N>(v, s, r);
+    else if constexpr (STEP == 1) gl::mul_2p32_n<N>(v, r);
+    else gl::mul_pow2_hi_n<N>(v, s, r);
+#pragma unroll
+    for (int i = 0; i < N; i++) x[idx[I0 + i]] = r[i];
+    __builtin_amdgcn_sched_barrier(0);
+    apply_pow2<STEP, CNT, I0 + N>(x, idx, sh);
+  } else {
+#pragma unroll
+    for (int i = I0; i < CNT; i++) {
+      if constexpr (STEP == 0) x[idx[i]] = gl::mul_pow2_lo(x[idx[i]], sh[i]);
+      else if constexpr (STEP == 1) x[idx[i]] = gl::mul_2p32(x[idx[i]]);
+      else x[idx[i]] = gl::mul_pow2_hi(x[idx[i]], sh[i]);
+    }
+  }
+}
+template <int S, bool DIF>
+__device__ __forceinline__ void dft16_twiddles(uint64_t (&x)[16]) {
+  constexpr Pow2Plan p = pow2_plan(S, DIF);
+  apply_pow2<0, p.n_lo>(x, p.lo_idx, p.lo_sh);
+  apply_pow2<1, p.n_mid>(x, p.mid_idx, p.lo_sh);
+  apply_pow2<2, p.n_hi>(x, p.hi_idx, p.hi_sh);
+}
+template <int H>
+__device__ __forceinline__ void dft16_addsub(uint64_t (&x)[16]) {
+#pragma unroll
+  for (int k0 = 0; k0 < 8; k0 += 4) {
+    uint64_t a[4], b[4], hi[4], lo[4];
+#pragma unroll
+    for (int i = 0; i < 4; i++) {
+      const int k = k0 + i, m = (k / H) * 2 * H + (k % H);
+      a[i] = x[m];
+      b[i] = x[m + H];
+    }
+    gl::canon_n<4>(b);
+    gl::add_n<4>(a, b, hi);
+    gl::sub_n<4>(a, b, lo);
+#pragma unroll
+    for (int i = 0; i < 4; i++) {
+      const int k = k0 + i, m = (k / H) * 2 * H + (k % H);
+      x[m] = hi[i];
+      x[m + H] = lo[i];
+    }
+    __builtin_amdgcn_sched_barrier(0);
+  }
+}
+template <int M0>
+__device__ __forceinline__ void layer16_load(uint64_t (&w)[4], const uint64_t* __restrict__ lay, uint32_t j, uint32_t log_sub) {
+#pragma unroll
+  for (int i = 0; i < 4; i++)
+    if (M0 + i < 16) w[i] = lay[((uint32_t)(16 + brev4(M0 + i)) << log_sub) + j];
+}
+template <int M0 = 1>
+__device__ __forceinline__ void layer16(uint64_t (&x)[16], const uint64_t* __restrict__ lay, uint32_t j, uint32_t log_sub,
+                                        const uint64_t (&w)[4]) {
+  uint64_t wn[4] = {0, 0, 0, 0};
+  if constexpr (M0 + 4 < 16) layer16_load<M0 + 4>(wn, lay, j, log_sub);
+  if constexpr (M0 + 4 <= 16) {
+    const uint64_t v[4] = {x[M0], x[M0 + 1], x[M0 + 2], x[M0 + 3]};
+    uint64_t r[4];
+    gl::mul_n<4>(v, w, r);
+#pragma unroll
+    for (int i = 0; i < 4; i++) x[M0 + i] = r[i];
+  } else {
+    const uint64_t v[3] = {x[13], x[14], x[15]}, w3[3] = {w[0], w[1], w[2]};
+    uint64_t r[3];
+    gl::mul_n<3>(v, w3, r);
+#pragma unroll
+    for (int i = 0; i < 3; i++) x[13 + i] = r[i];
+  }
+  __builtin_amdgcn_sched_barrier(0);
+  if constexpr (M0 + 4 < 16) layer16<M0 + 4>(x, lay, j, log_sub, wn);
+}
+__device__ __forceinline__ void layer16(uint64_t (&x)[16], const uint64_t* __restrict__ lay, uint32_t j, uint32_t log_sub) {
+  uint64_t w[4];
+  layer16_load<1>(w, lay, j, log_sub);
+  layer16<1>(x, lay, j, log_sub, w);
+}
+template <bool J0 = false>
+__device__ __forceinline__ void dit16(uint64_t (&x)[16], const uint64_t* __restrict__ lay, uint32_t j, uint32_t log_sub) {
+  if constexpr (!J0) layer16(x, lay, j, log_sub);
+  dft16_addsub<1>(x);
+  dft16_twiddles<1, false>(x);
+  dft16_addsub<2>(x);
+  dft16_twiddles<2, false>(x);
+  dft16_addsub<4>(x);
+  dft16_twiddles<3, false>(x);
+  dft16_addsub<8>(x);
+  uint64_t y[16];
+#pragma unroll
+  for (int q = 0; q < 16; q++) y[q] = x[(13 * q) & 15];
+#pragma unroll
+  for (int q = 0; q < 16; q++) x[q] = y[q];
+}
+template <bool J0 = false>
+__device__ __forceinline__ void dif16(uint64_t (&x)[16], const uint64_t* __restrict__ lay, uint32_t j, uint32_t log_sub) {
+  dft16_addsub<8>(x);
+  dft16_twiddles<0, true>(x);
+  dft16_addsub<4>(x);
+  dft16_twiddles<1, true>(x);
+  dft16_addsub<2>(x);
+  dft16_twiddles<2, true>(x);
+  dft16_addsub<1>(x);
+  uint64_t y[16];
+#pragma unroll
+  for (int m = 0; m < 16; m++) y[m] = x[brev4((3 * brev4(m)) & 15)];
+#pragma unroll
+  for (int m = 0; m < 16; m++) x[m] = y[m];
+  if constexpr (!J0) layer16(x, lay, j, log_sub);
 }
 
 template <int LOGR, bool DIF>
@@ -305,7 +337,13 @@
 }
 template <int R, int SH, bool CONTIG, bool DIF>
 __device__ __forceinline__ void sub_butterflies(uint64_t (&x)[16], const uint64_t* __restrict__ tw, uint32_t j,
-                                                uint32_t j_step_log, uint32_t log_sub, uint32_t tw_shift) {
+                                                uint32_t j_step_log, uint32_t log_sub, uint32_t tw_shift,
+                                                const uint64_t* __restrict__ lay) {
+  if constexpr (R == 4) {
+    if (DIF) dif16<CONTIG>(x, lay, j, log_sub);
+    else dit16<CONTIG>(x, lay, j, log_sub);
+    return;
+  }
   constexpr int G = 16 >> R;
 #pragma unroll
   for (int g = 0; g < G; g++) {
@@ -333,6 +371,7 @@
   uint64_t out_scalar;
   uint32_t log_n_total, n_cosets, n_units;
   const uint64_t* tw_top;
+  const uint64_t* lay;
 };
 
 
@@ -382,7 +421,7 @@
 #pragma unroll
     for (int m = 0; m < 16; m++) x[m] = src[m * T + t];
   }
-  dif_butterflies<4>(x, a.tw, t, L - 4, 0);
+  dif16(x, a.lay, t, L - 4);
 #pragma unroll
   for (int m = 0; m < 16; m++) buf[swz<L>(m * T + t)] = x[m];
   __syncthreads();
@@ -390,7 +429,7 @@
   for (int b = L - 8; b > 0; b -= 4) {
 #pragma unroll
     for (int m = 0; m < 16; m++) x[m] = buf[swz<L>(insert4(t, m, b))];
-    dif_butterflies<4>(x, a.tw, t & ((1u << b) - 1), b, L - (b + 4));
+    dif16(x, a.lay, t & ((1u << b) - 1), b);
 #pragma unroll
     for (int m = 0; m < 16; m++) buf[swz<L>(insert4(t, m, b))] = x[m];
     __syncthreads();
@@ -398,7 +437,7 @@
   const uint32_t base = gl::bitrev(t, L - 4) << 4;
 #pragma unroll
   for (int m = 0; m < 16; m++) x[m] = buf[swz<L>(base | m)];
-  sub_butterflies<RT, 0, true, true>(x, a.tw, 0, 0, 0, L - RT);
+  sub_butterflies<RT, 0, true, true>(x, a.tw, 0, 0, 0, L - RT, a.lay);
 #pragma unroll
   for (int m = 0; m < 16; m++) buf[swz<L>(base | m)] = x[m];
   __syncthreads();
@@ -509,7 +548,7 @@
   __syncthreads();
 #pragma unroll
   for (int m = 0; m < 16; m++) x[m] = buf[swz<L>(base | m)];
-  dit_butterflies<4, true>(x, tw, 0, 0, L - 4);
+  dit16<true>(x, a.lay, 0, 0);
 #pragma unroll
   for (int m = 0; m < 16; m++) buf[swz<L>(base | m)] = x[m];
   __syncthreads();
@@ -517,7 +556,7 @@
   for (int b = 4; b + 4 <= L - RT; b += 4) {
 #pragma unroll
     for (int m = 0; m < 16; m++) x[m] = buf[swz<L>(insert4(t, m, b))];
-    dit_butterflies<4>(x, tw, t & ((1u << b) - 1), b, L - (b + 4));
+    dit16(x, a.lay, t & ((1u << b) - 1), b);
 #pragma unroll
     for (int m = 0; m < 16; m++) buf[swz<L>(insert4(t, m, b))] = x[m];
     __syncthreads();
@@ -526,7 +565,7 @@
   asm volatile("" : "+v"(t2));
 #pragma unroll
   for (int m = 0; m < 16; m++) x[m] = buf[swz<L>(m * T + t2)];
-  sub_butterflies<RT, 4 - RT, false, false>(x, tw, t2, L - 4, L - RT, 0);
+  sub_butterflies<RT, 4 - RT, false, false>(x, tw, t2, L - 4, L - RT, 0, a.lay);
   uint64_t* dst = a.out + col * a.out_stride + coset * a.out_coset_stride + off;
 #pragma unroll
   for (int m0 = 0; m0 < 16; m0 += 4) {
@@ -601,7 +640,7 @@
     uint64_t x[16];
 #pragma unroll
     for (int m = 0; m < 16; m++) x[m] = buf[swz<L>(base | m)];
-    dit_butterflies<4, true>(x, tw, 0, 0, L - 4);
+    dit16<true>(x, a.lay, 0, 0);
 #pragma unroll
     for (int m = 0; m < 16; m++) buf[swz<L>(base | m)] = x[m];
     __syncthreads();
@@ -610,7 +649,7 @@
       asm volatile("" : "+v"(tc));
 #pragma unroll
       for (int m = 0; m < 16; m++) x[m] = buf[swz<L>(insert4(tc, m, b))];
-      dit_butterflies<4>(x, tw, tc & ((1u << b) - 1), b, L - (b + 4));
+      dit16(x, a.lay, tc & ((1u << b) - 1), b);
 #pragma unroll
       for (int m = 0; m < 16; m++) buf[swz<L>(insert4(tc, m, b))] = x[m];
       __syncthreads();
@@ -623,7 +662,7 @@
     }
 #pragma unroll
     for (int m = 0; m < 16; m++) x[m] = buf[swz<L>(m * T + t2)];
-    sub_butterflies<RT, 4 - RT, false, false>(x, tw, t2, L - 4, L - RT, 0);
+    sub_butterflies<RT, 4 - RT, false, false>(x, tw, t2, L - 4, L - RT, 0, a.lay);
     uint64_t* dst = a.out + col * a.out_stride + coset * a.out_coset_stride + off;
 #pragma unroll
     for (int m0 = 0; m0 < 16; m0 += 4) {
@@ -742,6 +781,13 @@
   uint32_t e = blockIdx.x * blockDim.x + threadIdx.x;
   if (e < count) out[e] = gl::pow(w, e);
 }
+__global__ void layer_table_kernel(uint64_t* out, uint32_t log_n, uint64_t w) {
+  const uint32_t idx = blockIdx.x * blockDim.x + threadIdx.x;
+  if (idx >= (2u << log_n)) return;
+  if (idx < 16) { out[idx] = 1; return; }
+  const uint32_t b = 31 - __clz(idx) - 4, r = (idx >> b) - 16, j = idx & ((1u << b) - 1);
+  out[idx] = gl::pow(w, (uint64_t)(j * r) << (log_n - b - 4));
+}
 __global__ void coset_scale_table_kernel(uint64_t* out, uint32_t log_n, uint32_t rate_bits, uint64_t w_m,
                                          int inverse) {
   uint32_t pos = blockIdx.x * blockDim.x + threadIdx.x;
@@ -781,14 +827,21 @@
   int dev = 0;
   BPG_HIP(hipGetDevice(&dev));
   std::lock_guard<std::mutex> lk(g_table_mu);
-  TableKey key{dev, kind, log_n, kind >= 2 ? rate_bits : 0};
+  TableKey key{dev, kind, log_n, (kind == 2 || kind == 3) ? rate_bits : 0};
   auto it = g_tables.find(key);
   if (it != g_tables.end()) {
     *out = it->second;
     return BP_OK;
   }
   uint64_t* d = nullptr;
-  if (kind >= 2) {
+  if (kind >= 4) {
+    if (log_n < 4 || log_n > LOG_BLK_MAX) return fail(BP_ERR_DEVICE, "radix-16 layer table for 2^%u points", log_n);
+    const uint32_t count = 2u << log_n;
+    BPG_HIP(hipMalloc(&d, (uint64_t)count * 8));
+    uint64_t w = gl::root(log_n);
+    if (kind == 5) w = gl::inv(w);
+    layer_table_kernel<<<ceil_div(count, 256), 256, 0, 0>>>(d, log_n, w);
+  } else if (kind >= 2) {
     uint64_t count = (uint64_t)1 << (log_n + rate_bits);
     BPG_HIP(hipMalloc(&d, count * 8));
     dim3 grid(ceil_div((uint64_t)1 << log_n, 256), 1u << rate_bits);
@@ -941,10 +994,11 @@
     src = out;
     src_stride = out_stride;
   }
-  if (log_blk >= 12) {
+  if (log_blk >= 12 && inverse) {
     Ntt16Args b{};
     b.in = src; b.in_stride = src_stride; b.out = out; b.out_stride = out_stride; b.out_coset_stride = 0;
     b.tw = tw_b; b.scale = nullptr; b.out_scalar = inverse ? gl::inv((uint64_t)1 << log_n) : 1;
+    if ((rc = get_table(5, log_blk, 0, &b.lay))) return rc;
     b.log_n_total = log_n; b.n_cosets = 1; b.n_units = 0;
     KernelTimer kt(PROF_INTT_DIF, st, 16.0 * (double)n_cols * (double)((uint64_t)1 << log_n));
     if (use_ntt_mx(log_blk, false)) {
@@ -994,8 +1048,9 @@
   const uint64_t *tw_n = nullptr, *tw_b = nullptr;
   int rc;
   if ((rc = get_table(inverse ? 1 : 0, log_blk, 0, &tw_b))) return rc;
-  if (log_blk >= 12) {
+  if (log_blk >= 12 && !inverse) {
     Ntt16Args b{};
+    if ((rc = get_table(4, log_blk, 0, &b.lay))) return rc;
     b.in = in; b.in_stride = in_stride; b.out = out; b.out_stride = out_stride; b.out_coset_stride = coset_stride;
     b.tw = tw_b; b.scale = scale; b.out_scalar = 1; b.log_n_total = log_n; b.n_cosets = n_cosets;
     b.n_units = n_cols << (log_n - log_blk);
diff --git a/proof_protocol_decoder_amd/csrc/stark_kernels.hip b/proof_protocol_decoder_amd/csrc/stark_kernels.hip
--- a/proof_protocol_decoder_amd/csrc/stark_kernels.hip
+++ b/proof_protocol_decoder_amd/csrc/stark_kernels.hip
@@ -1099,7 +1099,7 @@
 __global__ void __launch_bounds__(256) pow_grind_kernel(bpg::BatchOf<bpg::PowArgs> batch, unsigned long long* result) {
   const bpg::PowArgs& a = batch.a[blockIdx.z];
   result += blockIdx.z;
-  if (__hip_atomic_load(result, __ATOMIC_RELAXED, __HIP_MEMORY_SCOPE_AGENT) < a.base) return;
+  if (__hip_atomic_load(result, __ATOMIC_RELAXED, __HIP_MEMORY_SCOPE_AGENT) < a.base + blockIdx.x * (uint64_t)blockDim.x) return;
   const uint64_t cand = a.base + blockIdx.x * (uint64_t)blockDim.x + threadIdx.x;
   uint64_t s[12];
 #pragma unroll
@@ -1113,7 +1113,11 @@
 pow_grind_mx_kernel(bpg::BatchOf<bpg::PowArgs> batch, unsigned long long* result, const uint32_t* __restrict__ gtab) {
   const bpg::PowArgs& a = batch.a[blockIdx.z];
   result += blockIdx.z;
-  if (__hip_atomic_load(result, __ATOMIC_RELAXED, __HIP_MEMORY_SCOPE_AGENT) < a.base) return;
+  __shared__ uint32_t beaten;
+  if (threadIdx.x == 0)
+    beaten = __hip_atomic_load(result, __ATOMIC_RELAXED, __HIP_MEMORY_SCOPE_AGENT) < a.base + (uint64_t)blockIdx.x * 256;
+  __syncthreads();
+  if (beaten) return;
   constexpr int NG = GR ? GR : 2;
   __shared__ __attribute__((aligned(16))) uint32_t cin[GR ? poseidon::mx::CIN_GROUPED_WORDS<NG> : poseidon::mx::CIN_WORDS];
   __shared__ __attribute__((aligned(16))) uint32_t gt[GR ? poseidon::mx::grp::TABLE_WORDS<NG> : 4];
diff --git a/proof_protocol_decoder_amd/ops.py b/proof_protocol_decoder_amd/ops.py
--- a/proof_protocol_decoder_amd/ops.py
+++ b/proof_protocol_decoder_amd/ops.py
@@ -59,6 +59,14 @@
     n = a.numel()
     out = torch.empty((15, n), dtype=torch.int64, device=a.device)
     check(lib().bp_debug_field_ops(a.data_ptr(), b.data_ptr(), out.data_ptr(), n, _stream()))
+    return out
+
+
+def mul_pow2(a):
+    _require_cuda(a)
+    n = a.numel()
+    out = torch.empty((21, n), dtype=torch.int64, device=a.device)
+    check(lib().bp_debug_mul_pow2(a.data_ptr(), out.data_ptr(), n, _stream()))
     return out
 
 
```

Measured after the change: 34.30 (median of 6 runs). 1.3% higher.
